# gersteinlab/LESSeq

Hardware: AMD Instinct MI355X
Metric: MRF reads/sec through count+solve (higher is better)
Workload: dtype int32 coordinates / u64 counters (count), f64 (EM); 1 GPU; BASELINE configs[2]: 100M synthetic 100bp reads over 50k mixed events (SE/RI/A5SS/A3SS/MXE/AFE/ALE/T3), 24 chromosomes; events=50000

## Files before the change

include/lesseq_hip.h:

```cpp
#ifndef LESSEQ_HIP_H
#define LESSEQ_HIP_H

#include <stddef.h>
#include <stdint.h>

#ifdef __cplusplus
extern "C" {
#endif

#define LSQ_ABI_VERSION 2

typedef enum {
	LSQ_OK = 0,
	LSQ_E_ARG = -1,
	LSQ_E_IO = -2,
	LSQ_E_FORMAT = -3,
	LSQ_E_PARSE = -4,
	LSQ_E_RANGE = -5,
	LSQ_E_UNSUPPORTED = -6,
	LSQ_E_DEVICE = -7,
	LSQ_E_STATE = -8,
	LSQ_E_INTERNAL = -9,
	LSQ_E_TIMEOUT = -10
} lsq_status;
// ... 38 lines not shown
const char *lsq_events_chrom(const lsq_events *e, int64_t ev);
const char *lsq_events_strand(const lsq_events *e, int64_t ev);
int lsq_events_num_isoforms(const lsq_events *e, int64_t ev);
int lsq_events_num_segments(const lsq_events *e, int64_t ev);
const char *lsq_events_isoform_name(const lsq_events *e, int64_t ev, int iso);
int lsq_events_segment(const lsq_events *e, int64_t ev, int n, int64_t *start, int64_t *end);
uint64_t lsq_events_isoform_mask(const lsq_events *e, int64_t ev, int iso);
uint64_t lsq_events_isoform_length(const lsq_events *e, int64_t ev, int iso);
uint64_t lsq_events_ars(const lsq_events *e, int method, int64_t ev, int iso);
int lsq_events_span(const lsq_events *e, int64_t ev, int64_t *gene_start, int64_t *gene_end);
int64_t lsq_events_num_buckets(const lsq_events *e);
int64_t lsq_events_lds_table_bytes(const lsq_events *e);
int64_t lsq_events_host_genes(const lsq_events *e);
int lsq_events_set_shard(lsq_events *e, uint64_t first_event, uint64_t n_events);

int lsq_mrf_parse(const char *read_format, const char *path, lsq_events *e,
                  int n_threads, lsq_reads **out);
int lsq_reads_parse(const char *read_format, const char *path, lsq_events *e, int n_threads, lsq_reads **out);
#define LSQ_SAM_DEFAULT_SKIP_FLAGS 0x904u
#define LSQ_SAM_DEFAULT_MIN_MAPQ 0u
int lsq_sam_parse(const char *path, lsq_events *e, unsigned skip_flags, unsigned min_mapq, int n_threads, lsq_reads **out);
int lsq_sam_to_mrf(const void *sam_bytes, uint64_t len, unsigned skip_flags, unsigned min_mapq, char **mrf_text, uint64_t *mrf_len);
int lsq_bam_parse(const char *path, lsq_events *e, unsigned skip_flags, unsigned min_mapq, int n_threads, lsq_reads **out);
int lsq_bam_to_mrf(const void *bam_bytes, uint64_t len, unsigned skip_flags, unsigned min_mapq, char **mrf_text, uint64_t *mrf_len);
int lsq_bam_parse_checked(const char *path, lsq_events *e, unsigned skip_flags, unsigned min_mapq, int n_threads, lsq_reads **out);
int lsq_bam_to_mrf_checked(const void *bam_bytes, uint64_t len, unsigned skip_flags, unsigned min_mapq, char **mrf_text, uint64_t *mrf_len);
typedef struct { uint64_t file_bytes, blocks, inflated_bytes, header_lines, references, records, reads, read_blocks, blocks_repaired; } lsq_bam_report;
int lsq_bam_check_host(const char *path, int n_threads, lsq_bam_report *r);
int lsq_reads_wrap(uint64_t n_reads, const uint64_t *blk_off, const uint32_t *line_no,
                   const int32_t *blk_start, const int32_t *blk_end,
                   const uint16_t *blk_chrom_id, const uint8_t *blk_strand_id, lsq_reads **out);
void lsq_reads_free(lsq_reads *r);
uint64_t lsq_reads_count(const lsq_reads *r);
uint64_t lsq_reads_num_blocks(const lsq_reads *r);
int lsq_events_chrom_id(lsq_events *e, const char *chrom);
int lsq_events_strand_id(lsq_events *e, const char *strand);
const char *lsq_events_strand_name(const lsq_events *e, int strand_id);
int lsq_reads_arrays(const lsq_reads *r, const uint64_t **blk_off, const uint32_t **line_no,
                     const int32_t **blk_start, const int32_t **blk_end,
                     const uint16_t **blk_chrom_id, const uint8_t **blk_strand_id);


typedef struct lsq_ctx lsq_ctx;

int lsq_ctx_create(int device_id, lsq_ctx **out);
#define LSQ_CTX_LANES_IN_BACKGROUND 1u
int lsq_ctx_create_with(int device_id, unsigned flags, lsq_ctx **out);
void lsq_ctx_destroy(lsq_ctx *c);
void *lsq_ctx_stream(lsq_ctx *c);
int lsq_ctx_synchronize(lsq_ctx *c);
int lsq_ctx_synchronize_for(lsq_ctx *c, double seconds);

int lsq_events_upload(lsq_ctx *c, lsq_events *e);

int lsq_reads_upload(lsq_ctx *c, int method, const lsq_reads *r);
int lsq_reads_upload_mrf(lsq_ctx *c, int method, const char *read_format, const char *path);
typedef struct lsq_text lsq_text;
int lsq_text_stage(lsq_ctx *c, const char *path, lsq_text **out);
void lsq_text_free(lsq_text *t);
int lsq_reads_upload_text(lsq_ctx *c, int method, const char *read_format, lsq_text *t);
int lsq_text_stage_range(lsq_ctx *c, const char *path, uint64_t byte_begin, uint64_t byte_end, lsq_text **out);
int lsq_text_lines(lsq_ctx *c, lsq_text *t, uint64_t *n_newlines);
int lsq_reads_upload_text_at(lsq_ctx *c, int method, const char *read_format, lsq_text *t, int has_header, uint64_t first_line);
int lsq_mrf_parse_device(lsq_ctx *c, const char *read_format, const char *path, lsq_reads **out);
int lsq_last_mrf_timing(lsq_ctx *c, float *h2d_ms, float *parse_ms);
int lsq_ingest_stage_count(void);
const char *lsq_ingest_stage_name(int stage);
int lsq_last_ingest_stages(const lsq_ctx *c, float *ms, uint64_t *bytes, int capacity);
const char *lsq_last_ingest_stage_name(const lsq_ctx *c, int stage);
int lsq_last_ingest_stage_count(const lsq_ctx *c);
int lsq_last_sam_paths(const lsq_ctx *c, uint32_t *lines_listed, uint32_t *all_slow);
int lsq_last_bam_paths(const lsq_ctx *c, uint64_t *n_blocks, uint64_t *blocks_repaired);
int lsq_bam_check(lsq_ctx *c, const char *path, lsq_bam_report *r);
uint64_t lsq_reads_retained(const lsq_ctx *c, int method);
int lsq_last_library_report(const lsq_ctx *c, int method, uint64_t out[5]);
uint64_t lsq_reads_retained_blocks(const lsq_ctx *c, int method);
uint64_t lsq_reads_pooled(const lsq_ctx *c, int method);
uint64_t lsq_reads_pooled_blocks(const lsq_ctx *c, int method);
int lsq_reads_pool_format(const lsq_ctx *c, int method, int *compact, uint64_t *pool_bytes, uint64_t *pool_reads);

int lsq_count(lsq_ctx *c);
int lsq_count_status(lsq_ctx *c, uint32_t *exceptions, uint32_t *recounted);
int lsq_count_launch_info(lsq_ctx *c, uint32_t *reads_per_look, uint32_t *workgroups_per_cu);
int lsq_host_evaluated(const lsq_ctx *c, uint64_t *n_genes, uint64_t *n_reads);
int lsq_ctx_set_option(lsq_ctx *c, const char *name, double value);

int lsq_solve(lsq_ctx *c);

int64_t lsq_results_num_classes(const lsq_ctx *c);
int lsq_results_class_offsets(const lsq_ctx *c, uint64_t *class_off );
int lsq_results_counts(lsq_ctx *c, uint64_t *class_count, uint64_t *class_bases);
int lsq_results_set_counts(lsq_ctx *c, const uint64_t *class_count, const uint64_t *class_bases);
uint64_t lsq_counts_device_words(const lsq_ctx *c);
int lsq_counts_export_device(lsq_ctx *c, void *d_words);
int lsq_counts_import_device(lsq_ctx *c, const void *d_words);
int lsq_results_solve(lsq_ctx *c, double *theta, double *logll, uint32_t *em_iters, uint8_t *em_flags);
int lsq_solve_finalize(lsq_ctx *c, uint32_t *n_replayed);
int lsq_set_em_guard_band(lsq_ctx *c, double band);

int lsq_fim(lsq_ctx *c);
int64_t lsq_results_fim_size(const lsq_ctx *c);
int lsq_results_fim_offsets(const lsq_ctx *c, uint64_t *fim_off );
int lsq_results_fim(lsq_ctx *c, double *fim, double *var_by_diag, double *var_by_inverse);

int lsq_results_copy_device(lsq_ctx *c, void *d_class_count, void *d_theta, void *d_logll);
void *lsq_ctx_result_stream(lsq_ctx *c);

int lsq_shard_bounds(const lsq_events *e, int world, const double *weights ,
                     uint64_t *first , uint64_t *count );
uint64_t lsq_record_words(const lsq_events *e, uint64_t first, uint64_t count);
int lsq_results_pack_device(lsq_ctx *c, void *d_block);
int lsq_device_alloc(lsq_ctx *c, uint64_t bytes, void **out);
void lsq_device_free(lsq_ctx *c, void *p);
int lsq_device_read(lsq_ctx *c, void *host_dst, const void *device_src, uint64_t bytes);
int lsq_device_write(lsq_ctx *c, void *device_dst, const void *host_src, uint64_t bytes);
int lsq_gathered_unpack(const lsq_events *e, int world, const uint64_t *first, const uint64_t *count,
                        const uint64_t *blocks, uint64_t stride_words,
                        uint64_t *class_count, uint64_t *class_bases, double *theta, double *logll);
int lsq_results_device_order(const lsq_ctx *c, int32_t *dev2out );

int lsq_set_timing(lsq_ctx *c, int on);
int lsq_last_timing(lsq_ctx *c, float *count_ms, float *solve_ms);
int lsq_last_fast_kernel_ms(lsq_ctx *c, float *ms);


int lsq_format_count(const lsq_events *e, int n_methods, const uint64_t *class_count, char **out_text);
int lsq_format_solve(const lsq_events *e, int n_methods, const uint64_t *class_count,
                     const uint64_t *class_bases, const double *theta, const double *logll,
                     const double *total_read_bases, char **out_text);
void lsq_free(void *p);

int lsq_cli_run(const char *tool, int argc, const char *const *argv, char **out_text);
int lsq_cli_main(const char *tool, int argc, const char *const *argv);


int lsq_as_fisher(lsq_ctx *c, uint64_t n_tables, const double *cells , double *p);
int lsq_as_lrt(lsq_ctx *c, uint64_t n_rows, int n1, int n2, const double *count, const double *total ,
               double *stat, double *p);
int lsq_as_wilcox(lsq_ctx *c, uint64_t n_rows, int n1, int n2, const double *value , double *diff, double *p);
int lsq_as_adjust(lsq_ctx *c, uint64_t n, const double *p, double *p_bonferroni, double *p_bh);

typedef struct lsq_as_input lsq_as_input;
int lsq_as_read_matrix(const char *test, int n_paths, const char *const *paths, int n1, int n2, lsq_as_input **out);
int lsq_as_read_tables(const char *test, int n_paths, const char *const *paths, int n1, int n2, lsq_as_input **out);
void lsq_as_input_free(lsq_as_input *in);
uint64_t lsq_as_input_rows(const lsq_as_input *in);
int lsq_as_input_columns(const lsq_as_input *in);
const char *lsq_as_input_id(const lsq_as_input *in, uint64_t row);
const double *lsq_as_input_values(const lsq_as_input *in);
const double *lsq_as_input_totals(const lsq_as_input *in);
uint64_t lsq_as_input_left_out(const lsq_as_input *in);
int lsq_as_format_number(double v, char *buf, size_t cap);


typedef struct lsq_jn_index lsq_jn_index;
typedef struct lsq_jn_table lsq_jn_table;
int lsq_jn_index_build(const lsq_annotation *a, lsq_jn_index **out);
void lsq_jn_index_free(lsq_jn_index *ix);
int64_t lsq_jn_index_num_chroms(const lsq_jn_index *ix);
const char *lsq_jn_index_chrom_name(const lsq_jn_index *ix, int64_t chrom);
int64_t lsq_jn_index_num_introns(const lsq_jn_index *ix);
lsq_events *lsq_jn_index_dictionaries(lsq_jn_index *ix);
int lsq_jn_host(lsq_jn_index *ix, const char *read_format, const char *path, unsigned skip_flags, unsigned min_mapq,
                uint32_t min_overhang, int n_threads, lsq_jn_table **out);
int lsq_jn_host_reads(lsq_jn_index *ix, const lsq_reads *r, uint32_t min_overhang, int n_threads, lsq_jn_table **out);
int lsq_jn_device(lsq_ctx *c, lsq_jn_index *ix, const char *read_format, const char *path, uint32_t min_overhang, lsq_jn_table **out);
// ... 69 lines not shown
```

include/lesseq_hip_dev.h:

```cpp
#ifndef LESSEQ_HIP_DEV_H
#define LESSEQ_HIP_DEV_H

#include <stdint.h>
#include "lesseq_hip.h"

#ifdef __cplusplus
extern "C" {
#endif

int lsq_debug_counters(lsq_ctx *c, unsigned long long *out16);
int lsq_debug_wg_trace(lsq_ctx *c, unsigned long long *out, unsigned long long cap, unsigned long long *n, unsigned long long *n_workers);

int lsq_debug_slot_offsets(lsq_ctx *c, int method, unsigned long long *out, unsigned long long n);
int lsq_debug_plan_shares(const unsigned long long *slot_off, const unsigned char *packed, const unsigned long long *n1, const unsigned long long *n2,
                          const unsigned *look1, const unsigned *look2, unsigned long long n_buckets, unsigned long long grid,
                          const double *costs4, int weighted, int snap, unsigned long long *cuts);
int lsq_debug_offsets(lsq_ctx *c, int method, int which, unsigned long long *out, unsigned long long cap, unsigned long long *n);

int lsq_debug_set_em_order(lsq_ctx *c, const uint32_t *order, unsigned n_small_places, unsigned n_places);

int lsq_debug_stream_read_rate(lsq_ctx *c, unsigned long long bytes, double *gb_per_s);

int lsq_debug_throw(int kind);

int lsq_debug_last_parse_paths(const lsq_ctx *c, unsigned *tiles_handed, unsigned *lines_listed, unsigned *all_slow);

int lsq_debug_bgzf_inflate(lsq_ctx *c, const void *bytes, uint64_t len, void *out, uint64_t cap, uint64_t *n);

int lsq_debug_bgzf_crc32(lsq_ctx *c, const void *bytes, uint64_t len, uint32_t *crc, uint64_t cap, uint64_t *n);

int lsq_debug_hip_versions(int *compiled, int *runtime);

int64_t lsq_debug_events_covered(const lsq_events *e, const char *chrom, int minus, int64_t *starts, int64_t *ends, int64_t capacity);

#ifdef __cplusplus
}
#endif
#endif
```

lesseq_amd/_lib.py:

```python
import ctypes as C
import os

_HERE = os.path.dirname(os.path.abspath(__file__))
LIB_PATH = os.environ.get("LSQ_LIB") or os.path.join(_HERE, "_build", "liblesseq_hip.so")


class LsqError(RuntimeError):
    def __init__(self, status, msg):
        super().__init__("lsq status %d: %s" % (status, msg))
        self.status = status


if not os.path.exists(LIB_PATH):
    raise ImportError("%s is missing: build it with `make -C lesseq_amd/csrc` (or __graft_entry__.build()); "
                      "there is no fallback implementation" % LIB_PATH)

if os.environ.get("LSQ_NO_TORCH") != "1":
    try:
        import torch
    except Exception:
        pass

lib = C.CDLL(LIB_PATH)

# ... 32 lines not shown
_sig("lsq_events_compile_library", C.c_int, vp, C.c_int, P(cs), P(u64), C.c_int, P(vp))
_sig("lsq_events_library", C.c_int, vp)
_sig("lsq_library_from_name", C.c_int, cs)
_sig("lsq_debug_events_covered", C.c_int64, vp, cs, C.c_int, P(C.c_int64), P(C.c_int64), C.c_int64)
_sig("lsq_events_free", None, vp)
_sig("lsq_events_count", i64, vp)
_sig("lsq_events_total_isoforms", i64, vp)
_sig("lsq_events_gene_name", cs, vp, i64)
_sig("lsq_events_chrom", cs, vp, i64)
_sig("lsq_events_strand", cs, vp, i64)
_sig("lsq_events_num_isoforms", C.c_int, vp, i64)
_sig("lsq_events_num_segments", C.c_int, vp, i64)
_sig("lsq_events_isoform_name", cs, vp, i64, C.c_int)
_sig("lsq_events_segment", C.c_int, vp, i64, C.c_int, P(i64), P(i64))
_sig("lsq_events_isoform_mask", u64, vp, i64, C.c_int)
_sig("lsq_events_isoform_length", u64, vp, i64, C.c_int)
_sig("lsq_events_ars", u64, vp, C.c_int, i64, C.c_int)
_sig("lsq_events_span", C.c_int, vp, i64, P(i64), P(i64))
_sig("lsq_events_num_buckets", i64, vp)
_sig("lsq_events_lds_table_bytes", i64, vp)
_sig("lsq_events_host_genes", i64, vp)
_sig("lsq_events_set_shard", C.c_int, vp, u64, u64)
_sig("lsq_mrf_parse", C.c_int, cs, cs, vp, C.c_int, P(vp))
_sig("lsq_reads_parse", C.c_int, cs, cs, vp, C.c_int, P(vp))
_sig("lsq_sam_parse", C.c_int, cs, vp, C.c_uint, C.c_uint, C.c_int, P(vp))
_sig("lsq_sam_to_mrf", C.c_int, cs, u64, C.c_uint, C.c_uint, P(vp), P(u64))
_sig("lsq_bam_parse", C.c_int, cs, vp, C.c_uint, C.c_uint, C.c_int, P(vp))
_sig("lsq_bam_to_mrf", C.c_int, cs, u64, C.c_uint, C.c_uint, P(vp), P(u64))
_sig("lsq_bam_parse_checked", C.c_int, cs, vp, C.c_uint, C.c_uint, C.c_int, P(vp))
_sig("lsq_bam_to_mrf_checked", C.c_int, cs, u64, C.c_uint, C.c_uint, P(vp), P(u64))
_sig("lsq_bam_check_host", C.c_int, cs, C.c_int, P(BamReportStruct))
_sig("lsq_reads_wrap", C.c_int, u64, P(u64), P(u32), P(i32), P(i32), P(u16), P(u8), P(vp))
_sig("lsq_reads_free", None, vp)
_sig("lsq_reads_count", u64, vp)
_sig("lsq_reads_num_blocks", u64, vp)
_sig("lsq_events_chrom_id", C.c_int, vp, cs)
_sig("lsq_events_strand_id", C.c_int, vp, cs)
_sig("lsq_ctx_create", C.c_int, C.c_int, P(vp))
_sig("lsq_ctx_destroy", None, vp)
_sig("lsq_ctx_stream", vp, vp)
_sig("lsq_ctx_synchronize", C.c_int, vp)
_sig("lsq_ctx_synchronize_for", C.c_int, vp, C.c_double)
_sig("lsq_debug_throw", C.c_int, C.c_int)
_sig("lsq_debug_hip_versions", C.c_int, P(C.c_int), P(C.c_int))
_sig("lsq_events_upload", C.c_int, vp, vp)
_sig("lsq_reads_upload", C.c_int, vp, C.c_int, vp)
_sig("lsq_reads_arrays", C.c_int, vp, P(vp), P(vp), P(vp), P(vp), P(vp), P(vp))
_sig("lsq_events_strand_name", cs, vp, C.c_int)
_sig("lsq_reads_upload_mrf", C.c_int, vp, C.c_int, cs, cs)
_sig("lsq_text_stage", C.c_int, vp, cs, P(vp))
_sig("lsq_text_stage_range", C.c_int, vp, cs, u64, u64, P(vp))
_sig("lsq_text_lines", C.c_int, vp, vp, P(u64))
_sig("lsq_reads_upload_text_at", C.c_int, vp, C.c_int, cs, vp, C.c_int, u64)
_sig("lsq_results_set_counts", C.c_int, vp, P(u64), P(u64))
_sig("lsq_text_free", None, vp)
_sig("lsq_reads_upload_text", C.c_int, vp, C.c_int, cs, vp)
_sig("lsq_mrf_parse_device", C.c_int, vp, cs, cs, P(vp))
_sig("lsq_last_mrf_timing", C.c_int, vp, P(C.c_float), P(C.c_float))
_sig("lsq_set_log_level", None, C.c_int)
_sig("lsq_ingest_stage_count", C.c_int)
_sig("lsq_ingest_stage_name", cs, C.c_int)
_sig("lsq_last_ingest_stages", C.c_int, vp, P(C.c_float), P(u64), C.c_int)
_sig("lsq_last_ingest_stage_name", cs, vp, C.c_int)
_sig("lsq_last_sam_paths", C.c_int, vp, P(u32), P(u32))
_sig("lsq_last_ingest_stage_count", C.c_int, vp)
_sig("lsq_last_bam_paths", C.c_int, vp, P(u64), P(u64))
_sig("lsq_debug_bgzf_inflate", C.c_int, vp, cs, u64, vp, u64, P(u64))
_sig("lsq_debug_bgzf_crc32", C.c_int, vp, cs, u64, P(u32), u64, P(u64))
_sig("lsq_bam_check", C.c_int, vp, cs, P(BamReportStruct))
_sig("lsq_reads_retained", u64, vp, C.c_int)
_sig("lsq_last_library_report", C.c_int, vp, C.c_int, P(u64))
_sig("lsq_reads_retained_blocks", u64, vp, C.c_int)
_sig("lsq_reads_pooled", u64, vp, C.c_int)
_sig("lsq_reads_pooled_blocks", u64, vp, C.c_int)
_sig("lsq_reads_pool_format", C.c_int, vp, C.c_int, C.POINTER(C.c_int), C.POINTER(C.c_uint64), C.POINTER(C.c_uint64))
_sig("lsq_count", C.c_int, vp)
_sig("lsq_solve", C.c_int, vp)
_sig("lsq_results_num_classes", i64, vp)
_sig("lsq_results_class_offsets", C.c_int, vp, P(u64))
_sig("lsq_results_counts", C.c_int, vp, P(u64), P(u64))
_sig("lsq_results_solve", C.c_int, vp, P(C.c_double), P(C.c_double), P(u32), P(u8))
_sig("lsq_count_status", C.c_int, vp, P(u32), P(u32))
_sig("lsq_count_launch_info", C.c_int, vp, P(u32), P(u32))
_sig("lsq_host_evaluated", C.c_int, vp, P(u64), P(u64))
_sig("lsq_counts_device_words", u64, vp)
_sig("lsq_counts_export_device", C.c_int, vp, vp)
_sig("lsq_counts_import_device", C.c_int, vp, vp)
_sig("lsq_ctx_set_option", C.c_int, vp, cs, C.c_double)
_sig("lsq_solve_finalize", C.c_int, vp, P(u32))
_sig("lsq_set_em_guard_band", C.c_int, vp, C.c_double)
_sig("lsq_results_copy_device", C.c_int, vp, vp, vp, vp)
_sig("lsq_ctx_result_stream", vp, vp)
_sig("lsq_shard_bounds", C.c_int, vp, C.c_int, P(C.c_double), P(u64), P(u64))
_sig("lsq_record_words", u64, vp, u64, u64)
_sig("lsq_results_pack_device", C.c_int, vp, vp)
_sig("lsq_gathered_unpack", C.c_int, vp, C.c_int, P(u64), P(u64), P(u64), u64, P(u64), P(u64), P(C.c_double), P(C.c_double))
_sig("lsq_device_alloc", C.c_int, vp, u64, P(vp))
_sig("lsq_device_free", None, vp, vp)
_sig("lsq_device_read", C.c_int, vp, vp, vp, u64)
_sig("lsq_device_write", C.c_int, vp, vp, vp, u64)
_sig("lsq_results_device_order", C.c_int, vp, P(i32))
_sig("lsq_fim", C.c_int, vp)
_sig("lsq_results_fim_size", C.c_int64, vp)
_sig("lsq_results_fim_offsets", C.c_int, vp, P(C.c_uint64))
_sig("lsq_results_fim", C.c_int, vp, P(C.c_double), P(C.c_double), P(C.c_double))
_sig("lsq_set_timing", C.c_int, vp, C.c_int)
_sig("lsq_last_fast_kernel_ms", C.c_int, vp, P(C.c_float))
_sig("lsq_last_timing", C.c_int, vp, P(C.c_float), P(C.c_float))
_sig("lsq_format_count", C.c_int, vp, C.c_int, P(u64), P(vp))
_sig("lsq_format_solve", C.c_int, vp, C.c_int, P(u64), P(u64), P(C.c_double), P(C.c_double), P(C.c_double), P(vp))
_sig("lsq_cli_run", C.c_int, cs, C.c_int, P(cs), P(vp))
_sig("lsq_synth_write", C.c_int, P(SynthSpecStruct), cs, cs, C.c_int)
_sig("lsq_synth_write_sam", C.c_int, P(SynthSpecStruct), cs, cs)
_sig("lsq_as_fisher", C.c_int, vp, u64, P(C.c_double), P(C.c_double))
_sig("lsq_as_lrt", C.c_int, vp, u64, C.c_int, C.c_int, P(C.c_double), P(C.c_double), P(C.c_double), P(C.c_double))
_sig("lsq_as_wilcox", C.c_int, vp, u64, C.c_int, C.c_int, P(C.c_double), P(C.c_double), P(C.c_double))
_sig("lsq_as_adjust", C.c_int, vp, u64, P(C.c_double), P(C.c_double), P(C.c_double))
_sig("lsq_as_read_matrix", C.c_int, cs, C.c_int, P(cs), C.c_int, C.c_int, P(vp))
_sig("lsq_as_read_tables", C.c_int, cs, C.c_int, P(cs), C.c_int, C.c_int, P(vp))
_sig("lsq_as_input_free", None, vp)
_sig("lsq_as_input_rows", u64, vp)
_sig("lsq_as_input_columns", C.c_int, vp)
_sig("lsq_as_input_id", cs, vp, u64)
_sig("lsq_as_input_values", P(C.c_double), vp)
_sig("lsq_as_input_totals", P(C.c_double), vp)
_sig("lsq_as_input_left_out", u64, vp)
_sig("lsq_as_format_number", C.c_int, C.c_double, C.c_char_p, C.c_size_t)
_sig("lsq_synth_reads", C.c_int, P(SynthSpecStruct), vp, C.c_int, P(vp))
_sig("lsq_le_load_matrices", C.c_int, cs, cs, P(vp))
_sig("lsq_le_load_annotation", C.c_int, cs, cs, cs, cs, P(vp))
_sig("lsq_le_graphs_free", None, vp)
_sig("lsq_le_num_genes", i64, vp)
_sig("lsq_le_gene_name", cs, vp, i64)
_sig("lsq_le_gene_shape", C.c_int, vp, i64, P(C.c_int), P(C.c_int))
_sig("lsq_le_gene_positions", i64, vp, i64, P(P(i32)))
_sig("lsq_le_detect", C.c_int, vp, vp, P(vp))
_sig("lsq_le_result_free", None, vp)
_sig("lsq_le_type_name", cs, C.c_int)
_sig("lsq_le_num_events", i64, vp, C.c_int)
_sig("lsq_le_event", C.c_int, vp, C.c_int, i64, P(i64), P(i32))
_sig("lsq_le_format", C.c_int, vp, C.c_int, P(vp), P(vp))
_sig("lsq_le_result_times", C.c_int, vp, P(C.c_double))
_sig("lsq_le_write", C.c_int, vp, cs)
_sig("lsq_gtf_parse", C.c_int, vp, cs, P(vp))
_sig("lsq_gtf_parse_text", C.c_int, vp, cs, u64, P(vp))
_sig("lsq_gtf_free", None, vp)
_sig("lsq_gtf_num_transcripts", i64, vp)
_sig("lsq_gtf_num_genes", i64, vp)
_sig("lsq_gtf_num_exon_lines", i64, vp)
_sig("lsq_gtf_transcript_name", cs, vp, i64)
_sig("lsq_gtf_transcript_chrom", cs, vp, i64)
_sig("lsq_gtf_transcript_strand", cs, vp, i64)
_sig("lsq_gtf_transcript_exons", i64, vp, i64, P(P(i32)), P(P(i32)))
_sig("lsq_gtf_format", C.c_int, vp, P(vp), P(vp))
_sig("lsq_gtf_result_times", C.c_int, vp, P(C.c_double))
_sig("lsq_gtf_isoform_map", C.c_int, cs, u64, P(vp))
_sig("lsq_le_load_gtf", C.c_int, vp, cs, P(vp))
_sig("lsq_jn_index_build", C.c_int, vp, P(vp))
_sig("lsq_jn_index_free", None, vp)
_sig("lsq_jn_index_num_chroms", i64, vp)
_sig("lsq_jn_index_chrom_name", cs, vp, i64)
_sig("lsq_jn_index_num_introns", i64, vp)
_sig("lsq_jn_index_dictionaries", vp, vp)
_sig("lsq_jn_host", C.c_int, vp, cs, cs, C.c_uint, C.c_uint, u32, C.c_int, P(vp))
_sig("lsq_jn_host_reads", C.c_int, vp, vp, u32, C.c_int, P(vp))
_sig("lsq_jn_device", C.c_int, vp, vp, cs, cs, u32, P(vp))
# ... 36 lines not shown
```

lesseq_amd/api.py:

```python
import os
import ctypes as C

import numpy as np

from ._lib import lib, check, check_runtime_once, SynthSpecStruct, BamReportStruct, u64, u32, i32, u16, u8, i64, vp, cs, P

EVENT_TYPES = ("SE", "RI", "A5SS", "A3SS", "MXE", "AFE", "ALE", "T3")


def _b(s):
    return s.encode() if isinstance(s, str) else s


def _take_text(ptr):
    if not ptr:
        return ""
    s = C.string_at(ptr).decode()
    lib.lsq_free(ptr)
    return s


def _ptr(a, ct):
    return a.ctypes.data_as(P(ct))

# ... 327 lines not shown
            out = (u32 * cap)()
            st = lib.lsq_debug_bgzf_crc32(self.h, data, len(data), out, cap, C.byref(n))
            if st == -5 and n.value > cap:
                cap = n.value
                continue
            check(st)
            return [int(v) for v in out[:n.value]]

    def bam_check(self, path):
        r = BamReportStruct()
        check(lib.lsq_bam_check(self.h, _b(path), C.byref(r)))
        return _bam_report(r)

    def mrf_timing(self):
        a, b = C.c_float(), C.c_float()
        check(lib.lsq_last_mrf_timing(self.h, C.byref(a), C.byref(b)))
        return {"h2d_ms": a.value, "parse_ms": b.value}

    def parse_paths(self):
        a, b, c = C.c_uint(), C.c_uint(), C.c_uint()
        lib.lsq_debug_last_parse_paths.argtypes = [vp, P(C.c_uint), P(C.c_uint), P(C.c_uint)]
        lib.lsq_debug_last_parse_paths.restype = C.c_int
        check(lib.lsq_debug_last_parse_paths(self.h, C.byref(a), C.byref(b), C.byref(c)))
        return {"tiles_to_byte_walking_kernel": a.value, "lines_to_shared_splitter": b.value, "whole_file_byte_walking": bool(c.value)}

    def ingest_stages(self):
        n = lib.lsq_last_ingest_stage_count(self.h)
        ms, by = (C.c_float * n)(), (C.c_uint64 * n)()
        check(lib.lsq_last_ingest_stages(self.h, ms, by, n))
        return [{"stage": lib.lsq_last_ingest_stage_name(self.h, i).decode(), "ms": float(ms[i]), "bytes": int(by[i])} for i in range(n)]

    def retained(self, method):
        return lib.lsq_reads_retained(self.h, method)

    def library_report(self, method=0):
        out = (u64 * 5)()
        check(lib.lsq_last_library_report(self.h, method, out))
        return tuple(out)

    def pooled(self, method):
        return lib.lsq_reads_pooled(self.h, method)

    def pooled_blocks(self, method):
        return lib.lsq_reads_pooled_blocks(self.h, method)

    def pool_format(self, method):
        a, n = C.c_int(0), C.c_uint64(0)
        k = (C.c_uint64 * 3)()
        check(lib.lsq_reads_pool_format(self.h, method, C.byref(a), C.byref(n), k))
        return bool(a.value), n.value, tuple(int(x) for x in k)

    def retained_blocks(self, method):
        return lib.lsq_reads_retained_blocks(self.h, method)

    def count(self):
        check(lib.lsq_count(self.h))

    def solve(self):
        check(lib.lsq_solve(self.h))

    def set_option(self, name, value):
        check(lib.lsq_ctx_set_option(self.h, _b(name), float(value)))

    def count_status(self):
        M = max(self.events.n_methods, 1)
        e, r = (u32 * M)(), (u32 * M)()
        check(lib.lsq_count_status(self.h, e, r))
        return list(e)[:self.events.n_methods], list(r)[:self.events.n_methods]

    def counts_device_words(self):
        return int(lib.lsq_counts_device_words(self.h))

    def export_counts_device(self, d_ptr):
        check(lib.lsq_counts_export_device(self.h, vp(d_ptr)))

    def import_counts_device(self, d_ptr):
        check(lib.lsq_counts_import_device(self.h, vp(d_ptr)))

    def launch_info(self):
        a, b = u32(), u32()
        check(lib.lsq_count_launch_info(self.h, C.byref(a), C.byref(b)))
        return int(a.value), int(b.value)

    def set_em_guard_band(self, band):
        check(lib.lsq_set_em_guard_band(self.h, float(band)))

    def solve_finalize(self):
        n = u32()
        check(lib.lsq_solve_finalize(self.h, C.byref(n)))
        return n.value

    def synchronize(self):
        check(lib.lsq_ctx_synchronize(self.h))

    @property
    def stream(self):
        return lib.lsq_ctx_stream(self.h)

    def set_timing(self, on=True):
        check(lib.lsq_set_timing(self.h, 1 if on else 0))

    def timing(self):
        a, b = C.c_float(), C.c_float()
        check(lib.lsq_last_timing(self.h, C.byref(a), C.byref(b)))
        return a.value, b.value

    def copy_results_device(self, d_class_count=None, d_theta=None, d_logll=None):
        check(lib.lsq_results_copy_device(self.h, vp(d_class_count), vp(d_theta), vp(d_logll)))

    def pack_results_device(self, d_block):
        check(lib.lsq_results_pack_device(self.h, vp(d_block)))

    @property
    def result_stream(self):
        return lib.lsq_ctx_result_stream(self.h)

    def device_order(self):
        o = np.zeros(max(len(self.events), 1), np.int32)
        check(lib.lsq_results_device_order(self.h, _ptr(o, i32)))
        return o[:len(self.events)]

    def fast_kernel_ms(self):
        a = C.c_float()
        check(lib.lsq_last_fast_kernel_ms(self.h, C.byref(a)))
        return a.value

    def counts(self):
        n = lib.lsq_results_num_classes(self.h)
        M = self.events.n_methods
        cnt = np.zeros((max(M, 1), max(n, 1)), np.uint64)
        bases = np.zeros((max(M, 1), max(n, 1)), np.uint64)
        check(lib.lsq_results_counts(self.h, _ptr(cnt, u64), _ptr(bases, u64)))
        return cnt[:M, :n], bases[:M, :n]

    def set_counts(self, cnt, bases):
        cnt = np.ascontiguousarray(cnt, np.uint64)
        bases = np.ascontiguousarray(bases, np.uint64)
        check(lib.lsq_results_set_counts(self.h, _ptr(cnt, u64), _ptr(bases, u64)))

    def stage_text(self, path, byte_begin=0, byte_end=2 ** 64 - 1):
        h = vp()
        check(lib.lsq_text_stage_range(self.h, _b(path), byte_begin, byte_end, C.byref(h)))
        return h

    def text_lines(self, text):
        n = u64()
        check(lib.lsq_text_lines(self.h, text, C.byref(n)))
        return n.value

    def upload_reads_text(self, method, text, has_header=True, first_line=1, read_format="MRF_SINGLE", free=True):
        try:
            check(lib.lsq_reads_upload_text_at(self.h, method, _b(read_format), text, 1 if has_header else 0, first_line))
        finally:
            if free:
                lib.lsq_text_free(text)

    def solution(self):
        ne, ni = len(self.events), self.events.total_isoforms
        theta = np.zeros(max(ni, 1), np.float64)
        ll = np.zeros(max(ne, 1), np.float64)
        it = np.zeros(max(ne, 1), np.uint32)
        fl = np.zeros(max(ne, 1), np.uint8)
        check(lib.lsq_results_solve(self.h, _ptr(theta, C.c_double), _ptr(ll, C.c_double), _ptr(it, u32), _ptr(fl, u8)))
        return theta[:ni], ll[:ne], it[:ne], fl[:ne]

    def fim(self):
# ... 54 lines not shown
```

lesseq_amd/csrc/lsq_count.hip:

```cpp
#include "lsq_device.hpp"
#include <hip/hip_ext.h>

namespace {

#ifndef LSQ_COUNT_BLOCK
#define LSQ_COUNT_BLOCK 256
#endif
constexpr int COUNT_BLOCK = LSQ_COUNT_BLOCK;
constexpr unsigned long long BASES_MASK = (1ull << 40) - 1;

#ifdef LSQ_DEV
#define ABL(args, bits) ((((args).ablate) & (bits)) != 0u)
#else
#define ABL(args, bits) false
#endif


struct CountArgs {
	const BucketDesc *buckets;
	const unsigned char *images;
	const TieRec *ties;
	const unsigned char *strand_rank;
	const char *read_names; const unsigned long long *read_name_off;
	const char *gene_names; const unsigned *gene_name_off;
	unsigned n_buckets;
	unsigned ablate;
	unsigned tables_lds_bytes;
	const void *p1; const unsigned char *p1_strand; const unsigned *p1_line;
	const void *p2; const unsigned char *p2_strand; const unsigned *p2_line;
	unsigned compact;
	const unsigned *pn_blk_off; const unsigned *pn_nblk; const int2 *pn_se; const unsigned char *pn_strand; const unsigned *pn_line; const unsigned *pn_bucket;
	const unsigned long long *p1_off, *p2_off, *pn_off, *slot_off;
	const lsq::VisitRec *visits;
	const unsigned *wg_first;
	const unsigned long long *wg_cut;
	const lsq::WgPlan *wg_plan;
	unsigned long long *wg_trace;
	unsigned long long total_slots;
	unsigned long long n_pn;
	unsigned n_workers;
	unsigned long long *cnt, *bases;
	struct ExcEntry *exc;
	unsigned *exc_count;
	unsigned exc_cap;
	unsigned long long *dbg;
	unsigned long long *bar;
};

__device__ inline int2 unpack_one_block(const unsigned a, const int base) {
	const int s = base + (int)(a & lsq::COMPACT_OFF_MASK);
	return make_int2(s, s + (int)(a >> lsq::COMPACT_OFF_BITS));
}
__device__ inline int4 unpack_two_block(const unsigned a, const unsigned b, const int base) {
	const int s1 = base + (int)(a & lsq::COMPACT_OFF_MASK), e1 = s1 + (int)(a >> lsq::COMPACT_OFF_BITS);
	const int s2 = e1 + (int)(b & lsq::COMPACT_OFF_MASK);
	return make_int4(s1, e1, s2, s2 + (int)(b >> lsq::COMPACT_OFF_BITS));
}
__device__ inline int2 pool1_read(const CountArgs &A, const unsigned long long g, const int lo) {
	if (!A.compact) return reinterpret_cast<const int2 *>(A.p1)[g];
	return unpack_one_block(reinterpret_cast<const unsigned *>(A.p1)[g], lo - lsq::COMPACT_BIAS);
}
__device__ inline int4 pool2_read(const CountArgs &A, const unsigned long long g, const int lo) {
	if (!A.compact) return reinterpret_cast<const int4 *>(A.p2)[g];
	const uint2 v = reinterpret_cast<const uint2 *>(A.p2)[g];
	return unpack_two_block(v.x, v.y, lo - lsq::COMPACT_BIAS);
}

struct LdsView {
	const unsigned short *bins;
	const EventRec *ev;
	const int2 *segs;
	const unsigned *iso;
	unsigned long long *hist;
};

__device__ __noinline__ bool tie_orders_read_first(const CountArgs &A, unsigned ev_index, unsigned read_strand, unsigned line) {
	const TieRec *t = A.ties + ev_index;
	const unsigned rs = A.strand_rank[read_strand], gs = A.strand_rank[t->strand_id];
	if (rs != gs) return rs < gs;
	if (A.read_name_off) {
		const unsigned long long r0 = A.read_name_off[line], r1 = A.read_name_off[line + 1];
		const unsigned g0 = A.gene_name_off[ev_index], g1 = A.gene_name_off[ev_index + 1];
		const unsigned long long rn = r1 - r0;
		const unsigned gn = g1 - g0;
		for (unsigned long long i = 0; i < rn && i < gn; ++i) {
			const unsigned char a = (unsigned char)A.read_names[r0 + i], b = (unsigned char)A.gene_names[g0 + i];
			if (a != b) return a < b;
		}
		return rn < gn;
	}
	const unsigned mode = t->tie_mode;
	if (mode != 2) return mode == 1;
	unsigned pow10 = 1, nd = 1;
	while (nd < 10 && line / pow10 >= 10) { pow10 *= 10; ++nd; }
	const unsigned tl = t->tail_len;
	unsigned v = line;
	for (unsigned i = 0; i < nd && i < tl; ++i) {
		const unsigned char a = (unsigned char)('0' + v / pow10), b = (unsigned char)t->tail[i];
		if (a != b) return a < b;
		v %= pow10; pow10 /= 10;
	}
	return nd < tl;
}

struct Walk {
	int pos = 0, it = 0;
	bool found = false;
	unsigned mask = 0;
	int matched = 0;
	__device__ inline bool block(const int2 *segs, int nseg, int a, int b) {
		while (it < nseg) {
// ... 468 lines not shown
					const bool inside1 = v1 && !start1 && rd.y <= (int)cw1.z && rd.z != rd.y;
					const bool ends1 = inside1 && rd.y == (int)cw1.z;
					const unsigned ri = 3u * (v1 ? cx1.w : 0u);
					const uint4 w0r = C.recs[ri], w1r = C.recs[ri + 1u], w2r = C.recs[ri + 2u];
					const unsigned k2 = rd.z == (int)w1r.z ? 1u : (rd.z == (int)w2r.x ? 2u : (rd.z == (int)w2r.z ? 3u : 0u));
					const int end2 = k2 == 1u ? (int)w1r.w : (k2 == 2u ? (int)w2r.y : (int)w2r.w);
					const bool cont = ends1 && k2 > k1;
					const bool J = cont && rd.w <= end2;
					const bool S = inside1 && !cont;
					const bool drop = (v1 && start1 && rd.w <= (int)cw1.w) || (here && i1 == CELL_INFO_EMPTY);
					const unsigned len1 = (unsigned)(rd.y - rd.x), total = len1 + (unsigned)(rd.w - rd.z);
					const unsigned long long tbl = ((unsigned long long)w0r.w << 32) | w0r.z;
					const unsigned cls = (unsigned)(tbl >> (4u * ((1u << (k1 & 3u)) | (1u << k2)))) & 0xFu;
					const unsigned sa = cx1.x & 0xFFFFu;
					L.junction = cont;
					L.jslot = cls != 0u ? (w0r.y & 0xFFFFu) + cls - 1u : CELL_NONE;
					L.add = in && ((J && cls != 0u) || (S && sa != CELL_NONE && 50u * len1 > 49u * total));
					L.slot = J ? (w0r.y & 0xFFFFu) + cls - 1u : sa;
					L.matched = J ? total : len1;
					L.park = in && !(J || S || drop);
					L.hint = v1 ? (cx1.w | PARK_ONE_EVENT) : evf;
					L.c = make_int4((int)cw1.x, (int)cw1.y, 0, end2);
					if (ABL(A, 256u) && L.park) atomicAdd(&A.dbg[8 + (v1 ? 1 : 0)], 1ull);
					return L;
				};
				const uint4 u = cur[0];
				const int4 rd = make_int4((int)u.x, (int)u.y, (int)u.z, (int)u.w);
				const unsigned w0i = wt + lane * (unsigned)SW;
				const unsigned rel = w0i - first_rel;
				const bool in = w0i < ww1 && rel < n_rel;
				const Look L1 = look2(rd, in);
				unsigned n_add = L1.add ? 1u : 0u, s_add = L1.add ? L1.matched : 0u, n_add2 = 0, s_add2 = 0;
				park[0] = L1.park && !ABL(A, 17u | 1048576u);
				pe0[0] = uint4(u);
				pe1[0] = make_uint4(L1.hint, rel, 0u, 0u);
#pragma unroll
				for (int j = 1; j < N_READS; ++j) {
					const uint4 &v = cur[j];
					const int4 r2 = make_int4((int)v.x, (int)v.y, (int)v.z, (int)v.w);
					const unsigned wj = wt + lane * (unsigned)SW + (unsigned)j;
					const unsigned rel2 = wj - first_rel;
					const bool in2 = wj < ww1 && rel2 < n_rel;
					const bool same = in2 && L1.junction && r2.y == rd.y && r2.z == rd.z && L1.c.x <= r2.x && r2.x < L1.c.y && r2.w <= L1.c.w;
					n_add2 += (same && L1.jslot != CELL_NONE) ? 1u : 0u;
					s_add2 += (same && L1.jslot != CELL_NONE) ? (unsigned)((r2.y - r2.x) + (r2.w - r2.z)) : 0u;
					park[j] = in2 && !same && r2.y != r2.x && !ABL(A, 17u | 1048576u | 2097152u);
					pe0[j] = uint4(v);
					pe1[j] = make_uint4(PARK_EVENT_UNKNOWN, rel2, 0u, 0u);
				}
				if (!ABL(A, 1u)) {
					if (n_add && n_add2 && L1.slot == L1.jslot) { n_add += n_add2; s_add += s_add2; n_add2 = 0; }
					if (n_add) atomicAdd(&C.hist[L1.slot], ((unsigned long long)n_add << 40) | s_add);
					if (n_add2) atomicAdd(&C.hist[L1.jslot], ((unsigned long long)n_add2 << 40) | s_add2);
				} else asm volatile("" ::"v"(n_add), "v"(s_add), "v"(n_add2), "v"(s_add2));
			}
		}
		if (RPW == 1) {
			static_assert(RPW != 1 || N_READS == 2, "two parked entries a step");
#pragma unroll
			for (int q = 0; q < 2; ++q) {
				const bool pq = park[q ? N_READS - 1 : 0];
				const uint4 q0 = pe0[q ? N_READS - 1 : 0], q1 = pe1[q ? N_READS - 1 : 0];
				if (ABL(A, 256u) && pq) atomicAdd(&A.dbg[NB - 1], 1ull);
				R.push(pq, lane, q0, q1);
				if (R.live() >= 64u) {
					if (!ABL(A, 32u)) walk_parked<NB>(C, R, false);
					else R.head = R.tail;
				}
			}
		}
	};
	if (ww0 < ww1) fetch(ww0);
	for (unsigned wt = ww0; wt < ww1; wt += WAVES * TILE) {
		uint4 cur[SW];
#pragma unroll
		for (int k = 0; k < SW; ++k) cur[k] = nxt[k];
		if (wt + WAVES * TILE < ww1) fetch(wt + WAVES * TILE);
		do_step(cur, wt);
	}
	if (R.live() && !ABL(A, 32u)) walk_parked<NB>(C, R, true);
}


template <int NR>
__device__ inline void stream_pool1_compact(FastCtx &C, const uint4 *bins, const uint4 *cells, const uint4 *cellx, const unsigned n_cells, const BucketDesc &d,
                                            const CountArgs &A, uint4 *queue, const void *pool, const unsigned long long g0, const unsigned long long g1) {
	static_assert(NR == 4 || NR == 8, "one or two 16-byte words of four compact records");
	static_assert((unsigned)NR <= P1_GROUP_PAD, "a lane's records of a step lie in one cell group");
	constexpr int CW = NR / 4;
	constexpr unsigned TILE = 64u * NR;
	C.pool = 0u;
	C.slot0 = g0;
	global_words src = (global_words)pool;
	const unsigned lane = threadIdx.x & 63u, wave = (unsigned)__builtin_amdgcn_readfirstlane((int)(threadIdx.x >> 6));
	const unsigned long long R0 = g0 & ~(unsigned long long)(NR - 1);
	const unsigned n = (unsigned)(g1 - R0), first_rel = (unsigned)(g0 - R0), n_rel = (unsigned)(g1 - g0);
	const unsigned last_word = (n - 1u) >> 2;
	const int base = d.lo - lsq::COMPACT_BIAS;
	uint4 nxt[CW];
	auto fetch = [&](const unsigned t) {
#pragma unroll
		for (int cq = 0; cq < CW; ++cq) {
			const unsigned w = min((t >> 2) + lane * (unsigned)CW + (unsigned)cq, last_word);
			const u32x4 v = src[(R0 >> 2) + w];
			nxt[cq] = make_uint4(v.x, v.y, v.z, v.w);
		}
	};
	Ring<1> R;
	R.q = queue;
	const unsigned t_begin = min(wave * TILE, n);
	if (t_begin < n) fetch(t_begin);
	for (unsigned t = t_begin; t < n; t += WAVES * TILE) {
		unsigned rec[NR];
#pragma unroll
		for (int cq = 0; cq < CW; ++cq) { rec[4 * cq] = nxt[cq].x; rec[4 * cq + 1] = nxt[cq].y; rec[4 * cq + 2] = nxt[cq].z; rec[4 * cq + 3] = nxt[cq].w; }
		if (t + WAVES * TILE < n) fetch(t + WAVES * TILE);
		if (ABL(A, 512u)) {
#pragma unroll
			for (int j = 0; j < NR; ++j) asm volatile("" ::"v"(rec[j]));
			continue;
		}
		const int p0 = (int)(rec[0] & lsq::COMPACT_OFF_MASK) + base;
		const int rel0 = p0 - d.lo;
		const unsigned bin = rel0 <= 0 ? 0u : ((unsigned)rel0 >> d.shift);
		const uint4 br = bins[min(bin, d.n_bins - 1u)];
		unsigned ci = (br.x & 0xFFFFu) + (unsigned)(p0 >= (int)br.y) + (unsigned)(p0 >= (int)br.z) + (unsigned)(p0 >= (int)br.w);
		if (__any(p0 >= (int)br.w) && !ABL(A, 65536u)) {
			while (ci + 1u < n_cells && p0 >= (int)cells[ci + 1u].x) ++ci;
		}
		const unsigned cc = min(ci, n_cells - 1u);
		const uint4 cw = cells[cc];
		const uint4 cx = cellx[cc];
		const bool has = ci < n_cells && (int)cw.x <= p0 && p0 < (int)cw.y && !ABL(A, 8u);
		const bool both = has && (cx.z & CELLX_BOTH) != 0;
		const int e1 = has ? (int)cw.z - base : -1, e2 = has ? (int)cw.w - base : -1;
		const bool interior = t + TILE <= n && t >= first_rel;
		unsigned accN = 0, accA = 0, accL = 0;
		auto decide = [&](auto whole_step, auto one_threshold) {
#pragma unroll
			for (int j = 0; j < NR; ++j) {
				const unsigned len = rec[j] >> lsq::COMPACT_OFF_BITS;
				const int e = (int)(rec[j] & lsq::COMPACT_OFF_MASK) + (int)len;
				unsigned p = len | (min(len, 1u) << 24);
				if (!decltype(whole_step)::value) {
					const unsigned idx = t + lane * (unsigned)NR + (unsigned)j;
					p = (idx < n && idx - first_rel < n_rel) ? p : 0u;
				}
				accN += p;
				accA += e <= e1 ? p : 0u;
				if (!decltype(one_threshold)::value) accL += e <= e2 ? p : 0u;
			}
			if (decltype(one_threshold)::value) accL = accA;
		};
		if (__all(e1 == e2) && !ABL(A, 8388608u)) { if (interior) decide(std::true_type{}, std::true_type{}); else decide(std::false_type{}, std::true_type{}); }
		else { if (interior) decide(std::true_type{}, std::false_type{}); else decide(std::false_type{}, std::false_type{}); }
		const unsigned s1 = cx.x & 0xFFFFu, s2 = cx.x >> 16;
		if (!ABL(A, (1u | 16384u))) {
			const unsigned acc2 = both ? accL : accL - accA;
			if (accA && s1 != CELL_NONE) atomicAdd(&C.hist[s1], ((unsigned long long)(accA >> 24) << 40) | (accA & 0xFFFFFFu));
			if (acc2 && s2 != CELL_NONE) atomicAdd(&C.hist[s2], ((unsigned long long)(acc2 >> 24) << 40) | (acc2 & 0xFFFFFFu));
		} else asm volatile("" ::"v"(accA), "v"(accL));
		const bool lane_open = (accN >> 24) != ((both ? accA : accL) >> 24);
		if (ABL(A, 256u)) {
			const bool any_open = __any(lane_open);
			if (lane == 0) { atomicAdd(&A.dbg[12], 1ull); atomicAdd(&A.dbg[11], any_open ? 1ull : 0ull); }
		}
		if (__any(lane_open) && !ABL(A, 17u | 524288u)) {
#pragma unroll
			for (int h = 0; h < NR; h += 2) {
				uint4 en[2];
				unsigned open = 0;
#pragma unroll
				for (int j = h; j < h + 2; ++j) {
					const unsigned len = rec[j] >> lsq::COMPACT_OFF_BITS;
					const int so = (int)(rec[j] & lsq::COMPACT_OFF_MASK), e = so + (int)len;
					const unsigned idx = t + lane * (unsigned)NR + (unsigned)j, rel = idx - first_rel;
					const bool in = idx < n && rel < n_rel;
					const bool gone_near = both && (cx.z & CELLX_NEAR_NO_ABUT) != 0u && e > e1 && 50 * (e - e1) >= (int)len;
					const bool gone_far = both && (cx.z & CELLX_FAR_NO_ABUT) != 0u && e > e2 && 50 * (e - e2) >= (int)len;
					const bool done_near = e <= e1 || gone_near, done_far = e <= e2 || gone_far;
					const bool op = in && len != 0u && !(both ? (done_near && done_far) : e <= e2);
					open |= op ? 1u << (j - h) : 0u;
					const unsigned hint = !has ? PARK_EVENT_UNKNOWN : (!both ? (cx.w | PARK_ONE_EVENT) :
					                      (done_far ? (cx.w | PARK_ONE_EVENT) : (done_near ? ((cx.z & 0xFFFFu) | PARK_ONE_EVENT) : PARK_EVENT_UNKNOWN)));
					en[j - h] = make_uint4((unsigned)(so + base), (unsigned)(so + base) + len, hint, rel);
					if (ABL(A, 256u) && op) { atomicAdd(&A.dbg[5 + (has ? (both ? 2 : 1) : 0)], 1ull); atomicAdd(&A.dbg[0], 1ull); }
				}
				R.push2(open, lane, en[0], en[1]);
				if (R.live() >= 64u) {
					if (!ABL(A, 32u)) walk_parked<1, false>(C, R, false, base);
					else R.head = R.tail;
				}
			}
		}
	}
	if (R.live() && !ABL(A, 32u)) walk_parked<1, false>(C, R, true, base);
}

template <int NR>
__device__ inline void stream_pool2_compact(FastCtx &C, const uint4 *bins, const uint4 *cells, const uint4 *cellx, const unsigned n_cells, const BucketDesc &d,
                                            const CountArgs &A, uint4 *queue, const void *pool, const unsigned long long g0, const unsigned long long g1) {
	static_assert((NR == 2 || NR == 4 || NR == 8) && (unsigned)NR <= P2_GROUP_PAD, "whole 16-byte words of two compact records, inside one junction group");
	constexpr int CW = NR / 2;
	constexpr unsigned TILE = 64u * NR;
	C.pool = 1u;
	C.slot0 = g0;
	global_words src = (global_words)pool;
	const unsigned lane = threadIdx.x & 63u, wave = (unsigned)__builtin_amdgcn_readfirstlane((int)(threadIdx.x >> 6));
	const unsigned long long R0 = g0 & ~(unsigned long long)(NR - 1);
	const unsigned n = (unsigned)(g1 - R0), first_rel = (unsigned)(g0 - R0), n_rel = (unsigned)(g1 - g0);
	const unsigned last_word = (n - 1u) >> 1;
	const int base = d.lo - lsq::COMPACT_BIAS;
	uint4 nxt[CW];
	auto fetch = [&](const unsigned t) {
#pragma unroll
		for (int cq = 0; cq < CW; ++cq) {
			const unsigned w = min((t >> 1) + lane * (unsigned)CW + (unsigned)cq, last_word);
			const u32x4 v = src[(R0 >> 1) + w];
			nxt[cq] = make_uint4(v.x, v.y, v.z, v.w);
		}
	};
	Ring<1> R;
	R.q = queue;
	const unsigned t_begin = min(wave * TILE, n);
	if (t_begin < n) fetch(t_begin);
	for (unsigned t = t_begin; t < n; t += WAVES * TILE) {
		unsigned ra[NR], rb[NR];
#pragma unroll
		for (int cq = 0; cq < CW; ++cq) { ra[2 * cq] = nxt[cq].x; rb[2 * cq] = nxt[cq].y; ra[2 * cq + 1] = nxt[cq].z; rb[2 * cq + 1] = nxt[cq].w; }
		if (t + WAVES * TILE < n) fetch(t + WAVES * TILE);
		if (ABL(A, 512u)) {
#pragma unroll
			for (int j = 0; j < NR; ++j) asm volatile("" ::"v"(ra[j]), "v"(rb[j]));
			continue;
		}
		const bool interior = t + TILE <= n && t >= first_rel;
		const unsigned idx0 = t + lane * (unsigned)NR, rel0 = idx0 - first_rel;
		const bool in0 = interior || (idx0 < n && rel0 < n_rel);
		const int4 rd = unpack_two_block(ra[0], rb[0], base);
		const int rel_p = rd.x - d.lo;
		const unsigned bin = rel_p <= 0 ? 0u : ((unsigned)rel_p >> d.shift);
		const uint4 br = bins[min(bin, d.n_bins - 1u)];
		unsigned c1 = (br.x & 0xFFFFu) + (unsigned)(rd.x >= (int)br.y) + (unsigned)(rd.x >= (int)br.z) + (unsigned)(rd.x >= (int)br.w);
		const unsigned evf = br.x >> 16;
		if (__any(rd.x >= (int)br.w) && !ABL(A, 65536u)) {
			while (c1 + 1u < n_cells && rd.x >= (int)cells[c1 + 1u].x) ++c1;
		}
		const unsigned c1c = min(c1, n_cells - 1u);
		const uint4 cw1 = cells[c1c];
		const uint4 cx1 = cellx[c1c];
		const unsigned i1 = cx1.y;
		const unsigned k1 = (i1 >> 2) & 0x3Fu;
		const bool here = c1 < n_cells && (int)cw1.x <= rd.x && rd.x < (int)cw1.y && !ABL(A, 8u);
		const bool v1 = here && i1 < CELL_INFO_EMPTY;
		const bool start1 = k1 == CELL_K_START;
		const bool inside1 = v1 && !start1 && rd.y <= (int)cw1.z && rd.z != rd.y;
		const bool ends1 = inside1 && rd.y == (int)cw1.z;
		const bool ends1b = v1 && !start1 && (int)cw1.w > (int)cw1.z && rd.y == (int)cw1.w && rd.z != rd.y;
		const unsigned ri = 3u * (v1 ? cx1.w : 0u);
		const uint4 w0r = C.recs[ri], w1r = C.recs[ri + 1u], w2r = C.recs[ri + 2u];
		const unsigned k2 = rd.z == (int)w1r.z ? 1u : (rd.z == (int)w2r.x ? 2u : (rd.z == (int)w2r.z ? 3u : 0u));
		const int end2 = k2 == 1u ? (int)w1r.w : (k2 == 2u ? (int)w2r.y : (int)w2r.w);
		const unsigned abut = (w0r.y >> FAST_ABUT_SHIFT) & 7u;
		const bool abut2 = k2 != 0u && k2 < 3u && ((abut >> k2) & 1u) != 0u;
		const int end2b = !abut2 ? end2 : (k2 == 1u ? (int)w2r.y : (int)w2r.w);
		const unsigned k1e = ends1b ? k1 + 1u : k1;
		const bool junction = (ends1 || ends1b) && k2 > k1e;
		const bool J = junction && rd.w <= end2, Jb = junction && rd.w > end2 && rd.w <= end2b;
		const unsigned len1 = ra[0] >> lsq::COMPACT_OFF_BITS, total = len1 + (rb[0] >> lsq::COMPACT_OFF_BITS);
		const unsigned long long tbl = ((unsigned long long)w0r.w << 32) | w0r.z;
		const unsigned mask1 = (1u << (k1 & 3u)) | (ends1b ? 2u << (k1 & 3u) : 0u), maskA = mask1 | (1u << k2), maskB = maskA | (2u << k2);
		const unsigned clsA = (unsigned)(tbl >> (4u * (maskA & 15u))) & 0xFu, clsB = abut2 ? (unsigned)(tbl >> (4u * (maskB & 15u))) & 0xFu : 0u;
		const unsigned sa = cx1.x & 0xFFFFu;
		const unsigned slotA = clsA != 0u ? (w0r.y & 0xFFFFu) + clsA - 1u : CELL_NONE, slotB = clsB != 0u ? (w0r.y & 0xFFFFu) + clsB - 1u : CELL_NONE;
		const bool any_plain = __any(!junction);
		bool two = false, empty = false, near_free = false, far_free = false, S = false, drop = false, addS = false;
		int e1c = 0, e2c = 0;
// ... 67 lines not shown
		}
	}
	if (R.live() && !ABL(A, 32u)) walk_parked<2, true>(C, R, true, base);
}

__device__ inline void global_add_merged(unsigned long long *cnt, unsigned long long *bases, bool want, const unsigned slot, const unsigned matched) {
	const unsigned lane = threadIdx.x & 63u;
#pragma unroll 1
	for (int round = 0; round < 4; ++round) {
		const unsigned long long m = __ballot(want);
		if (!m) return;
		const unsigned lead = (unsigned)__ffsll((long long)m) - 1u;
		const unsigned s0 = (unsigned)__builtin_amdgcn_readlane((int)slot, lead);
		const bool same = want && slot == s0;
		const unsigned n = (unsigned)__popcll(__ballot(same));
		const unsigned sum = wave_sum_u32(same ? matched : 0u);
		if (lane == lead) { atomicAdd(&cnt[s0], (unsigned long long)n); atomicAdd(&bases[s0], (unsigned long long)sum); }
		want = want && !same;
	}
	if (want) { atomicAdd(&cnt[slot], 1ull); atomicAdd(&bases[slot], (unsigned long long)matched); }
}

__device__ inline void pool_n_worker(const CountArgs &A, const unsigned long long n_pn, const unsigned n_workers) {
	const unsigned long long gsz = (unsigned long long)n_workers * COUNT_BLOCK;
	for (unsigned long long g0 = (unsigned long long)blockIdx.x * COUNT_BLOCK; g0 < n_pn; g0 += gsz) {
		const unsigned long long g = g0 + threadIdx.x;
		bool active = g < n_pn;
		const unsigned b = active ? A.pn_bucket[g] : 0u;
		const BucketDesc *d = A.buckets + b;
		active = active && d->kind == 1;
		const unsigned *bins = reinterpret_cast<const unsigned *>(A.images + d->img_off);
		const uint4 *recs = reinterpret_cast<const uint4 *>(A.images + d->img_off + d->ev_off);
		const int2 *blk = A.pn_se + (active ? A.pn_blk_off[g] : 0u);
		const int nblk = active ? (int)A.pn_nblk[g] : 1;
		int p = 0, q = 0, total = 0;
		unsigned i = 0;
		if (active) {
			p = blk[0].x; q = blk[nblk - 1].y;
			for (int k = 0; k < nblk; ++k) total += blk[k].y - blk[k].x;
			const int rel = p - d->lo;
			const unsigned bin = rel <= 0 ? 0u : min((unsigned)rel >> d->shift, d->n_bins - 1u);
			i = bins[4u * bin] >> 16;
		}
		while (__any(active)) {
			bool want = false;
			unsigned slot = 0, matched = 0;
			if (active) {
				if (i >= d->n_events) active = false;
				else {
					const uint4 w0 = recs[3u * i];
					const int2 *segs = reinterpret_cast<const int2 *>(recs + 3u * i + 1u);
					const int gs = segs[0].x, ge = (int)w0.x;
					if (gs > p) active = false;
					else {
						bool cand = p <= ge;
						if (cand && p == gs) {
							if (q == ge) {
								const unsigned at = atomicAdd(A.exc_count, 1u);
								if (at < A.exc_cap) { ExcEntry e; e.slot = g; e.bucket = b; e.ev_pool_scan = i | (2u << 29); A.exc[at] = e; }
							}
							cand = q > ge;
						}
						if (cand) {
							const int nseg = (int)((w0.y >> FAST_NSEG_SHIFT) & 7u);
							Walk w;
							for (int k = 0; k < nblk; ++k) { const int2 bk = blk[k]; if (!w.block(segs, nseg, bk.x, bk.y)) break; }
							const unsigned long long tbl = ((unsigned long long)w0.w << 32) | w0.z;
							const unsigned cls = w.mask < 16u ? (unsigned)(tbl >> (4u * w.mask)) & 0xFu : 0u;
							if (cls != 0 && 50ll * w.matched > 49ll * total) { want = true; slot = d->cls_base + (w0.y & 0xFFFFu) + cls - 1; matched = (unsigned)w.matched; }
						}
						if (p <= ge && !(w0.y & FAST_FLAG_OVERLAPS_NEXT)) active = false;
						++i;
					}
				}
			}
			global_add_merged(A.cnt, A.bases, want, slot, matched);
		}
	}
}

#ifndef LSQ_FAST_WAVES
#define LSQ_FAST_WAVES 6
#endif
template <bool COMPACT, int P1W>
__global__ void __launch_bounds__(COUNT_BLOCK, P1W == 4 ? 5 : LSQ_FAST_WAVES) lsq_count_fast_kernel(CountArgs A) {
	extern __shared__ __align__(16) unsigned char lds[];
	const unsigned tid = threadIdx.x;
	struct Trace {
		unsigned long long *p;
		__device__ Trace(unsigned long long *q) : p(q) { if (p && threadIdx.x == 0) p[4u * blockIdx.x] = wall_clock64(); }
		__device__ ~Trace() { if (p && threadIdx.x == 0) p[4u * blockIdx.x + 1u] = wall_clock64(); }
	} trace(ABL(A, 4194304u) ? A.wg_trace : nullptr);
	if (blockIdx.x < A.n_workers) { pool_n_worker(A, A.n_pn, A.n_workers); return; }
	const unsigned wg = blockIdx.x - A.n_workers, n_wg = gridDim.x - A.n_workers;
	uint4 *wave_queue = reinterpret_cast<uint4 *>(lds + A.tables_lds_bytes) + (tid >> 6) * WAVE_QUEUE_WORDS;
	(void)n_wg;
	typedef const lsq::VisitRec __attribute__((address_space(4))) *const_visit;
	typedef const lsq::WgPlan __attribute__((address_space(4))) *const_plan;
	const_plan plan = (const_plan)(A.wg_plan + wg);
	const unsigned long long s_begin = plan->s_begin, s_end = plan->s_end;
	if (s_begin >= s_end) return;
	if (ABL(A, 4096u)) return;
	const_visit vr = &plan->first;
	unsigned b = vr->b;
	bool first_visit = true;
	while (b < A.n_buckets) {
		const unsigned long long bs = vr->bs;
		if (bs >= s_end) break;
		BucketDesc d;
		d.img_off = vr->d.img_off; d.img_bytes = vr->d.img_bytes; d.n_events = vr->d.n_events; d.n_bins = vr->d.n_bins; d.lo = vr->d.lo; d.shift = vr->d.shift;
		d.ev_off = vr->d.ev_off; d.seg_off = vr->d.seg_off; d.iso_off = vr->d.iso_off; d.hist_off = vr->d.hist_off; d.n_cls = vr->d.n_cls; d.cls_base = vr->d.cls_base;
		d.ev_base = vr->d.ev_base; d.chrom_id = vr->d.chrom_id; d.kind = vr->d.kind; d.hi = vr->d.hi;
		const unsigned long long be = vr->be, p1o = vr->p1o, n1 = vr->p1n, p2o = vr->p2o, n2 = vr->p2n;
		const unsigned next = vr->next;
		unsigned char *buf = lds;
		if (!first_visit) __syncthreads();
		first_visit = false;
		{
			global_words src = (global_words)(A.images + d.img_off);
			uint4 *dst = reinterpret_cast<uint4 *>(buf);
			for (unsigned i = tid; i < d.img_bytes / 16; i += COUNT_BLOCK) { const u32x4 t = src[i]; dst[i] = make_uint4(t.x, t.y, t.z, t.w); }
			unsigned long long *h = reinterpret_cast<unsigned long long *>(buf + d.hist_off);
			for (unsigned i = tid; i < HIST_REPLICAS * (d.n_cls | 1u); i += COUNT_BLOCK) h[i] = 0;
		}
		__syncthreads();
		if (ABL(A, 8192u)) return;
		const uint4 *bins = reinterpret_cast<const uint4 *>(buf);
		const uint4 *cells = reinterpret_cast<const uint4 *>(buf + d.seg_off);
		const unsigned n_cells = d.iso_off & 0xFFFFu;
		const uint4 *cellx = reinterpret_cast<const uint4 *>(buf + d.seg_off + 16u * (d.iso_off >> 16));
		FastCtx C;
		C.bins = bins; C.lo = d.lo; C.shift = d.shift; C.n_bins = d.n_bins;
		C.recs = reinterpret_cast<const uint4 *>(buf + d.ev_off);
		C.hist = reinterpret_cast<unsigned long long *>(buf + d.hist_off) + (tid & (HIST_REPLICAS - 1u)) * (d.n_cls | 1u);
		C.n_events = d.n_events; C.bucket = b;
		C.slot0 = 0; C.pool = 0;
		C.exc = A.exc; C.exc_count = A.exc_count; C.exc_cap = A.exc_cap; C.ablate = A.ablate; C.dbg = A.dbg;
		C.trace = (ABL(A, 4194304u) && A.wg_trace) ? A.wg_trace + 4u * blockIdx.x : nullptr;
		const unsigned long long l0 = (s_begin > bs ? s_begin : bs) - bs;
		const unsigned long long l1 = (s_end < be ? s_end : be) - bs;
		if (l0 < n1 && !ABL(A, 1024u)) {
			if constexpr (COMPACT) stream_pool1_compact<2 * P1W>(C, bins, cells, cellx, n_cells, d, A, wave_queue, A.p1, p1o + l0, p1o + (l1 < n1 ? l1 : n1));
			else stream_pool_wide<2>(C, bins, cells, cellx, n_cells, d, A, wave_queue, reinterpret_cast<const uint4 *>(A.p1), p1o + l0, p1o + (l1 < n1 ? l1 : n1));
		}
		if (l1 > n1 && l0 < n1 + n2 && !ABL(A, 2048u)) {
			const unsigned long long q0 = p2o + ((l0 > n1 ? l0 : n1) - n1), q1 = p2o + ((l1 < n1 + n2 ? l1 : n1 + n2) - n1);
			if constexpr (COMPACT) stream_pool2_compact<(P1W == 4 ? LSQ_P2_COMPACT_WORDS_W5 : LSQ_P2_COMPACT_WORDS)>(C, bins, cells, cellx, n_cells, d, A, wave_queue, A.p2, q0, q1);
			else stream_pool_wide<1>(C, bins, cells, cellx, n_cells, d, A, wave_queue, reinterpret_cast<const uint4 *>(A.p2), q0, q1);
		}
		__syncthreads();
		for (unsigned i = tid; i < d.n_cls; i += COUNT_BLOCK) {
			const unsigned long long *h0 = reinterpret_cast<const unsigned long long *>(buf + d.hist_off) + i;
			unsigned long long v = 0;
#pragma unroll
			for (unsigned r = 0; r < HIST_REPLICAS; ++r) v += h0[r * (d.n_cls | 1u)];
			if (v && !ABL(A, 4u)) {
				atomicAdd(&A.cnt[d.cls_base + i], v >> 40);
				atomicAdd(&A.bases[d.cls_base + i], v & BASES_MASK);
			}
		}
		if (be >= s_end) break;
		b = next;
		vr = (const_visit)(A.visits + b);
	}
}

struct GlobalBucket {
	const BucketDesc *d;
	const unsigned *bins;
	const uint4 *recs;
};

__device__ inline GlobalBucket global_bucket(const CountArgs &A, unsigned b) {
	GlobalBucket G;
	G.d = A.buckets + b;
	G.bins = reinterpret_cast<const unsigned *>(A.images + G.d->img_off);
	G.recs = reinterpret_cast<const uint4 *>(A.images + G.d->img_off + G.d->ev_off);
	return G;
}

__device__ void eval_read_global(const CountArgs &A, const GlobalBucket &G, const int2 *blk, int nblk, unsigned i, bool scan,
                                 unsigned strand_id, unsigned line) {
	const BucketDesc &d = *G.d;
	const int p = blk[0].x, q = blk[nblk - 1].y;
	int total = 0;
	for (int k = 0; k < nblk; ++k) total += blk[k].y - blk[k].x;
	for (; i < d.n_events; ++i) {
		const uint4 w0 = G.recs[3u * i], w1 = G.recs[3u * i + 1], w2 = G.recs[3u * i + 2];
		const int gs = (int)w1.x, ge = (int)w0.x;
		if (gs > p) break;
		bool cand = p <= ge;
		if (cand && p == gs) {
			if (q < ge) cand = false;
			else if (q == ge && tie_orders_read_first(A, d.ev_base + i, strand_id, line)) cand = false;
		}
		if (cand) {
			int2 segs[4] = {make_int2((int)w1.x, (int)w1.y), make_int2((int)w1.z, (int)w1.w), make_int2((int)w2.x, (int)w2.y), make_int2((int)w2.z, (int)w2.w)};
			const int nseg = (int)((w0.y >> FAST_NSEG_SHIFT) & 7u);
			Walk w;
			for (int k = 0; k < nblk; ++k) { const int2 bk = blk[k]; if (!w.block(segs, nseg, bk.x, bk.y)) break; }
			const unsigned long long tbl = ((unsigned long long)w0.w << 32) | w0.z;
			const unsigned cls = w.mask < 16u ? (unsigned)(tbl >> (4u * w.mask)) & 0xFu : 0u;
			if (cls != 0 && 50ll * w.matched > 49ll * total) {
				const unsigned slot = d.cls_base + (w0.y & 0xFFFFu) + cls - 1;
				atomicAdd(&A.cnt[slot], 1ull);
				atomicAdd(&A.bases[slot], (unsigned long long)(unsigned)w.matched);
			}
		}
		if (!scan) break;
		if (p <= ge && !(w0.y & FAST_FLAG_OVERLAPS_NEXT)) break;
	}
}

__device__ inline unsigned first_event_for(const GlobalBucket &G, int p) {
	const BucketDesc &d = *G.d;
	const int rel = p - d.lo;
	unsigned bin = rel <= 0 ? 0u : ((unsigned)rel >> d.shift);
	bin = min(bin, d.n_bins - 1u);
	return G.bins[4u * bin] >> 16;
}

__device__ void recount_all_reads(const CountArgs &A, unsigned long long n_pn);

__global__ void __launch_bounds__(256) lsq_count_cleanup_kernel(const CountArgs *Ap, int force_recount, unsigned long long n_pn,
                                                                const ExcEntry *exc, const unsigned *exc_count, unsigned exc_cap) {
// ... 89 lines not shown
	}
	for (size_t b = 0; b <= B; ++b) cum_b[b] = cum[std::min<size_t>(bseg[b], S)];
	const double total_cost = cum[S];
	const double wsum = (double)grid * (1.0 + taper) / 2.0;
	auto part_before = [&](unsigned long long g) {
		const double k = (double)g, slope = grid > 1 ? (taper - 1.0) / (double)(grid - 1) : 0.0;
		return (k + slope * k * (k - 1.0) / 2.0) / wsum;
	};
	size_t bb = 0, si = 0;
	for (unsigned long long g = 1; g < grid && total_cost > 0; ++g) {
		const double tc = total_cost * part_before(g), share = total_cost * (part_before(g + 1) - part_before(g));
		while (bb + 1 < B && cum_b[bb + 1] <= tc) ++bb;
		while (si + 1 < S && cum[si + 1] <= tc) ++si;
		const double xb = tc - cum_b[bb], yb = cum_b[bb + 1] - tc;
		unsigned long long t;
		if (pc.snap && xb <= yb && xb < 0.3 * share) t = so[bb];
		else if (pc.snap && yb < xb && yb < 0.3 * share) t = so[bb + 1];
		else {
			const double r = tc - cum[si] - jump[si];
			const unsigned long long len = x[si + 1] - x[si];
			t = x[si] + (r <= 0.0 ? 0ull : std::min<unsigned long long>((unsigned long long)(r / dens[si]), len));
		}
		cut[(size_t)g] = std::max(t, cut[(size_t)g - 1]);
	}
	if (!(total_cost > 0)) for (unsigned long long g = 1; g < grid; ++g) cut[(size_t)g] = total_slots * g / grid;
	cut[(size_t)grid] = total_slots;
	for (unsigned long long g = 0; g < grid; ++g)
		if (cut[(size_t)g + 1] - cut[(size_t)g] > (1ull << 21)) {
			for (unsigned long long q = 1; q < grid; ++q) cut[(size_t)q] = total_slots * q / grid;
			break;
		}
}

void plan_share_cuts(const unsigned long long *so, const unsigned char *visited_kind, const unsigned long long *pn1, const unsigned long long *pn2,
                     const unsigned *look1, const unsigned *look2, const size_t B, const unsigned long long grid, const SharePlanCosts &pc, unsigned long long *cut) {
	if (!(pc.weighted && pn1 && pn2 && look1 && look2)) { plan_share_cuts_seg(so, visited_kind, B, nullptr, nullptr, nullptr, nullptr, 0, grid, pc, cut); return; }
	std::vector<unsigned long long> x; std::vector<unsigned char> kind; std::vector<unsigned> looks, bseg(B + 1, 0);
	for (size_t b = 0; b < B; ++b) {
		bseg[b] = (unsigned)kind.size();
		const unsigned long long ns = so[b + 1] - so[b];
		if (!ns) continue;
		const bool visited = visited_kind[b] != 0;
		const unsigned long long n1 = visited ? std::min(pn1[b], ns) : 0, n2 = visited ? std::min(pn2[b], ns - n1) : 0;
		if (n1) { x.push_back(so[b]); kind.push_back(0); looks.push_back(look1[b]); }
		if (n2) { x.push_back(so[b] + n1); kind.push_back(1); looks.push_back(look2[b]); }
		if (ns - n1 - n2) { x.push_back(so[b] + n1 + n2); kind.push_back(2); looks.push_back(0); }
	}
	bseg[B] = (unsigned)kind.size();
	x.push_back(B ? so[B] : 0);
	plan_share_cuts_seg(so, visited_kind, B, x.data(), kind.data(), looks.data(), bseg.data(), kind.size(), grid, pc, cut);
}

int run_count(lsq_ctx *c) {
	const lsq_events &E = *c->E;
	const size_t n_cls = E.n_cls_total;
	const int M = E.n_methods;
	hipStream_t st_em = nullptr;
	const int set = c->flip ^ 1, other = c->flip;
	hipStream_t st = c->opt_two_count_streams ? c->stream_count2[set] : c->stream;
	if (c->mark_recorded2[set]) HIP_TRY(hipStreamWaitEvent(st, c->ev_mark2[set], 0));
	HIP_TRY(hipMemsetAsync(c->counters.p + (size_t)other * c->counters_per_set, 0, c->counters_per_set * sizeof(unsigned long long), c->stream_em2[other]));
	HIP_TRY(hipEventRecord(c->ev_mark2[other], c->stream_em2[other]));
	c->mark_recorded2[other] = true;
	select_counter_set(c, set);
	st_em = c->stream_em;
	c->fast_launched = 0;
	struct Cleanup { CountArgs A; unsigned long long n_pn; int m; };
	std::vector<Cleanup> cleanups;
	bool counted_signalled = false;
	if (c->time_events) HIP_TRY(hipEventRecord(c->ev0, st));
	const unsigned generic_tables_bytes = (std::max<unsigned>(E.max_lds_bytes, 16) + 15u) & ~15u;
	const unsigned tables_bytes = generic_tables_bytes;
	double max_skew = 0.0;
	for (int m = 0; m < M; ++m) max_skew = std::max(max_skew, c->reads[m].skew);
	const unsigned cap = c->opt_wg_per_cu >= 0 ? (unsigned)c->opt_wg_per_cu : (c->em_small_places >= c->opt_em_flat_min && max_skew < 4.0 ? 5u : 0u);
	const unsigned lds_bytes = std::max(tables_bytes + WAVES * WAVE_QUEUE_WORDS * 16, cap ? 160u * 1024u / (cap + 1u) + 16u : 0u);
	if (lds_bytes > 160 * 1024) return fail(LSQ_E_UNSUPPORTED, "bucket tables + read tile exceed the CU's LDS");
	bool all_compact = true;
	for (int m = 0; m < M; ++m) if (c->reads[m].total_slots && !c->reads[m].compact) all_compact = false;
	const int p1w = !all_compact ? 2 : (c->opt_reads_per_look ? (c->opt_reads_per_look == 8 ? 4 : 2) : (cap != 0 && cap <= 5 ? 4 : 2));
	const void *const fn_wide = (const void *)lsq_count_fast_kernel<false, 2>;
	const void *const fn_compact = p1w == 4 ? (const void *)lsq_count_fast_kernel<true, 4> : (const void *)lsq_count_fast_kernel<true, 2>;
	c->last_reads_per_look = 2u * (unsigned)p1w;
	if (lds_bytes > 64 * 1024) {
		HIP_TRY(hipFuncSetAttribute(fn_wide, hipFuncAttributeMaxDynamicSharedMemorySize, (int)lds_bytes));
		HIP_TRY(hipFuncSetAttribute(fn_compact, hipFuncAttributeMaxDynamicSharedMemorySize, (int)lds_bytes));
		HIP_TRY(hipFuncSetAttribute((const void *)lsq_count_generic_kernel, hipFuncAttributeMaxDynamicSharedMemorySize, (int)lds_bytes));
	}
	unsigned per_cu = std::max(1u, std::min(2048u / COUNT_BLOCK, (160u * 1024u) / lds_bytes));
	{
		if (c->occ_lds_bytes != lds_bytes || c->occ_p1w != p1w) {
			int nb = 0;
			int nb2 = 0;
			HIP_TRY(hipOccupancyMaxActiveBlocksPerMultiprocessor(&nb, fn_wide, (int)COUNT_BLOCK, (size_t)lds_bytes));
			HIP_TRY(hipOccupancyMaxActiveBlocksPerMultiprocessor(&nb2, fn_compact, (int)COUNT_BLOCK, (size_t)lds_bytes));
			c->occ_lds_bytes = lds_bytes; c->occ_p1w = p1w; c->occ_blocks = all_compact ? nb2 : std::min(nb, nb2);
		}
		if (c->occ_blocks >= 1) per_cu = std::min(per_cu, (unsigned)c->occ_blocks);
	}
	c->last_wg_per_cu = per_cu;
	for (int m = 0; m < M; ++m) {
		MethodReads &mr = c->reads[m];
		if (mr.total_slots == 0 || E.buckets.empty()) continue;
		const double mult = c->opt_grid_mult > 0 ? c->opt_grid_mult : (mr.skew >= 32.0 ? 4.0 : (mr.skew >= 4.0 || p1w == 4 ? 3.0 : 2.0));
		unsigned long long grid = (unsigned long long)((double)c->n_cu * per_cu * mult);
		grid = std::max(grid, mr.total_slots / (1ull << 21) + 1);
		grid = std::min<unsigned long long>(grid, std::max<unsigned long long>(mr.total_slots / 64, 1));
#ifdef LSQ_DEV
		if (const char *e = getenv("LSQ_GRID_WGS")) { const long v = atol(e); if (v >= 1) grid = (unsigned long long)v; }
#endif
		if (mr.wg_grid != grid) {
			const std::vector<unsigned long long> &so = mr.slot_off_host;
			const size_t B = E.buckets.size();
			std::vector<unsigned long long> cut((size_t)grid + 1, 0);
			std::vector<unsigned> first((size_t)grid, 0);
			const bool weighted = c->opt_share_weighted && mr.plan_n1.size() == B && mr.plan_park1.size() == B;
			SharePlanCosts pc;
			pc.weighted = weighted; pc.snap = c->opt_snap_shares;
			pc.two_block = c->opt_share_cost_p2; pc.walk_look = c->opt_share_cost_park; pc.visit = c->opt_share_cost_visit;
			pc.taper = c->opt_share_taper > 0 ? c->opt_share_taper : (mr.skew >= 4.0 ? 0.25 : 0.5);
			pc.hot = c->opt_share_cost_hot;
			std::vector<unsigned char> visited(B, 0);
			for (size_t q = 0; q < B; ++q) visited[q] = E.buckets[q].kind == 1u ? 1 : 0;
			if (weighted && mr.plan_seg_x.size() >= 2 && mr.plan_seg_first.size() == B + 1)
				plan_share_cuts_seg(so.data(), visited.data(), B, mr.plan_seg_x.data(), mr.plan_seg_kind.data(), mr.plan_seg_looks.data(), mr.plan_seg_first.data(),
				                    mr.plan_seg_kind.size(), grid, pc, cut.data());
			else
				plan_share_cuts(so.data(), visited.data(), weighted ? mr.plan_n1.data() : nullptr, weighted ? mr.plan_n2.data() : nullptr,
				                weighted ? mr.plan_park1.data() : nullptr, weighted ? mr.plan_park2.data() : nullptr, B, grid, pc, cut.data());
			size_t bb = 0;
			for (unsigned long long g = 0; g < grid; ++g) {
				while (bb + 1 < B && so[bb + 1] <= cut[(size_t)g]) ++bb;
				const unsigned f = mr.next_packed_host[bb];
				first[(size_t)g] = (f < B && so[f] < cut[(size_t)g + 1]) ? f : (unsigned)B;
			}
			int rc = mr.wg_first.upload(first.data(), first.size(), st);
			if (!rc) rc = mr.wg_cut.upload(cut.data(), cut.size(), st);
			if (rc) return rc;
			{
				std::vector<WgPlan> plan((size_t)grid);
				for (unsigned long long g = 0; g < grid; ++g) {
					WgPlan &w = plan[(size_t)g];
					w.s_begin = cut[(size_t)g]; w.s_end = cut[(size_t)g + 1];
					w.first = mr.visits_host[std::min<size_t>(first[(size_t)g], B)];
				}
				if ((rc = mr.wg_plan.upload(plan.data(), plan.size(), st))) return rc;
				HIP_TRY(hipStreamSynchronize(st));
			}
			HIP_TRY(hipStreamSynchronize(st));
			mr.wg_grid = grid;
		}
		CountArgs A{};
		A.buckets = c->buckets.p; A.images = c->images.p; A.ties = c->ties.p; A.strand_rank = c->strand_rank.p;
		A.wg_first = mr.wg_first.p; A.wg_cut = mr.wg_cut.p; A.wg_plan = mr.wg_plan.p; A.visits = mr.visits.p;
		A.read_names = mr.named ? mr.names.p : nullptr; A.read_name_off = mr.named ? mr.name_off.p : nullptr;
		A.gene_names = c->gene_names.p; A.gene_name_off = c->gene_name_off.p;
		A.n_buckets = (unsigned)E.buckets.size();
		A.tables_lds_bytes = tables_bytes;
		A.ablate = c->dev_ablate;
		A.compact = mr.compact ? 1u : 0u;
		A.p1 = mr.p1.p; A.p1_strand = mr.p1_strand.p; A.p1_line = mr.p1_line.p;
		A.p2 = mr.p2.p; A.p2_strand = mr.p2_strand.p; A.p2_line = mr.p2_line.p;
		A.pn_blk_off = mr.pn_blk_off.p; A.pn_nblk = mr.pn_nblk.p; A.pn_se = reinterpret_cast<const int2 *>(mr.pn_se.p);
		A.pn_strand = mr.pn_strand.p; A.pn_line = mr.pn_line.p; A.pn_bucket = mr.pn_bucket.p;
		A.p1_off = mr.p1_off.p; A.p2_off = mr.p2_off.p; A.pn_off = mr.pn_off.p; A.slot_off = mr.slot_off.p;
		A.total_slots = mr.total_slots;
		A.cnt = c->cnt.p + (size_t)m * n_cls; A.bases = c->bases.p + (size_t)m * n_cls;
		A.exc = mr.exc.p + (size_t)set * mr.exc_cap; A.exc_count = c->exc_count.p + 2 * m; A.exc_cap = (unsigned)mr.exc_cap;
		A.dbg = c->dbg.p; A.bar = c->dbg.p + 16 + m;
		A.wg_trace = nullptr;
		const unsigned long long n_pn = mr.pn_strand.n;
		A.n_pn = n_pn;
		const unsigned workers_per_cu = 2;
		A.n_workers = (unsigned)std::min<unsigned long long>((n_pn + COUNT_BLOCK - 1) / COUNT_BLOCK, (unsigned long long)c->n_cu * workers_per_cu);
#ifdef LSQ_DEV
		if (c->dev_ablate & 32768u) A.n_workers = 0;
#endif
		if (c->has_fast) {
			if (c->time_events) HIP_TRY(hipEventRecord(c->evf0[m], st));
			const bool last_streaming = m == M - 1 && !c->has_generic && !c->time_events;
			const dim3 fgrid((unsigned)grid + A.n_workers);
#ifdef LSQ_DEV
			if (c->dev_ablate & 4194304u) {
				if (c->wg_trace.n < 4ull * fgrid.x) { int rc = c->wg_trace.alloc(4ull * fgrid.x); if (rc) return rc; }
				HIP_TRY(hipMemsetAsync(c->wg_trace.p, 0, 4ull * fgrid.x * sizeof(unsigned long long), st));
				c->wg_trace_n = fgrid.x; c->wg_trace_workers = A.n_workers;
				A.wg_trace = c->wg_trace.p;
			}
#endif
			void *kargs[] = {(void *)&A};
			HIP_TRY(hipExtLaunchKernel(mr.compact ? fn_compact : fn_wide, fgrid, dim3(COUNT_BLOCK), kargs, lds_bytes, st, nullptr, last_streaming ? c->ev_counted2[set] : nullptr, 0));
			if (last_streaming) counted_signalled = true;
			if (c->time_events) HIP_TRY(hipEventRecord(c->evf1[m], st));
			c->fast_launched |= 1 << m;
			cleanups.push_back({A, n_pn, m});
		}
		if (c->has_generic) {
			hipLaunchKernelGGL(lsq_count_generic_kernel, dim3((unsigned)grid), dim3(COUNT_BLOCK), generic_tables_bytes, st, A);
			HIP_TRY(hipGetLastError());
		}
	}
	if (c->time_events) HIP_TRY(hipEventRecord(c->ev1, st));
	c->count_timed = c->time_events;
	if (!counted_signalled) HIP_TRY(hipEventRecord(c->ev_counted2[set], st));
	HIP_TRY(hipStreamWaitEvent(st_em, c->ev_counted2[set], 0));
	const unsigned rgrid = std::max(16u, (unsigned)c->n_cu);
	if (c->recount_args.n < 2 * (size_t)LSQ_MAX_METHODS * sizeof(CountArgs)) {
		int rc = c->recount_args.alloc(2 * (size_t)LSQ_MAX_METHODS * sizeof(CountArgs));
		if (rc) return rc;
		c->recount_args_host.assign(2 * (size_t)LSQ_MAX_METHODS * sizeof(CountArgs), 0);
	}
	for (const Cleanup &u : cleanups) {
		const size_t slot = ((size_t)set * LSQ_MAX_METHODS + (size_t)u.m) * sizeof(CountArgs);
		if (memcmp(c->recount_args_host.data() + slot, &u.A, sizeof(CountArgs)) != 0) {
			memcpy(c->recount_args_host.data() + slot, &u.A, sizeof(CountArgs));
			HIP_TRY(hipMemcpyAsync(c->recount_args.p + slot, c->recount_args_host.data() + slot, sizeof(CountArgs), hipMemcpyHostToDevice, st_em));
		}
		const CountArgs *dA = reinterpret_cast<const CountArgs *>(c->recount_args.p + slot);
		hipLaunchKernelGGL(lsq_count_cleanup_kernel, dim3(c->opt_cleanup_grid ? c->opt_cleanup_grid : rgrid), dim3(256), 0, st_em, dA, c->opt_recount ? 1 : 0, u.n_pn,
		                   (const ExcEntry *)u.A.exc, (const unsigned *)u.A.exc_count, u.A.exc_cap);
		HIP_TRY(hipGetLastError());
	}
	return LSQ_OK;
}

}

extern "C" {

int lsq_count_status(lsq_ctx *c, uint32_t *exceptions, uint32_t *recounted) LSQ_API_TRY {
	if (!c) return fail(LSQ_E_ARG, "null context");
	if (!c->counted) return fail(LSQ_E_STATE, "lsq_count must come first");
	HIP_TRY(hipSetDevice(c->device));
	{ int rc = sync_all(c); if (rc) return rc; }
	std::vector<unsigned> h(c->exc_count.n);
	HIP_TRY(hipMemcpy(h.data(), c->exc_count.p, h.size() * sizeof(unsigned), hipMemcpyDeviceToHost));
	note_overflow(c, h);
	for (int m = 0; m < c->E->n_methods; ++m) {
		if (exceptions) exceptions[m] = h[2 * (size_t)m];
		if (recounted) recounted[m] = h[2 * (size_t)m + 1];
	}
	return LSQ_OK;
} LSQ_API_CATCH

int lsq_count_launch_info(lsq_ctx *c, uint32_t *reads_per_look, uint32_t *workgroups_per_cu) LSQ_API_TRY {
	if (!c) return fail(LSQ_E_ARG, "null context");
	if (!c->counted) return fail(LSQ_E_STATE, "lsq_count must come first");
	if (reads_per_look) *reads_per_look = c->last_reads_per_look;
	if (workgroups_per_cu) *workgroups_per_cu = c->last_wg_per_cu;
	return LSQ_OK;
} LSQ_API_CATCH

int lsq_debug_counters(lsq_ctx *c, unsigned long long *out8) LSQ_API_TRY {
	HIP_TRY(hipSetDevice(c->device));
	{ int rc = sync_all(c); if (rc) return rc; }
	HIP_TRY(hipMemcpy(out8, c->dbg.p, 16 * sizeof(unsigned long long), hipMemcpyDeviceToHost));
	std::vector<unsigned> h(c->exc_count.n);
	HIP_TRY(hipMemcpy(h.data(), c->exc_count.p, h.size() * sizeof(unsigned), hipMemcpyDeviceToHost));
	out8[4] = h[0];
	return LSQ_OK;
} LSQ_API_CATCH

int lsq_debug_wg_trace(lsq_ctx *c, unsigned long long *out, unsigned long long cap, unsigned long long *n, unsigned long long *n_workers) LSQ_API_TRY {
	HIP_TRY(hipSetDevice(c->device));
	{ int rc = sync_all(c); if (rc) return rc; }
	const unsigned long long k = std::min<unsigned long long>(cap, c->wg_trace_n);
	if (k) HIP_TRY(hipMemcpy(out, c->wg_trace.p, 4 * k * sizeof(unsigned long long), hipMemcpyDeviceToHost));
	*n = k; *n_workers = c->wg_trace_workers;
	return LSQ_OK;
} LSQ_API_CATCH

int lsq_debug_plan_shares(const unsigned long long *slot_off, const unsigned char *packed, const unsigned long long *n1, const unsigned long long *n2,
                          const unsigned *look1, const unsigned *look2, unsigned long long n_buckets, unsigned long long grid,
                          const double *costs4, int weighted, int snap, unsigned long long *cuts) LSQ_API_TRY {
	if (!slot_off || !packed || !costs4 || !cuts || grid == 0) return fail(LSQ_E_ARG, "null argument");
	lsq::SharePlanCosts pc;
	pc.weighted = weighted != 0; pc.snap = snap != 0;
	pc.two_block = costs4[0]; pc.walk_look = costs4[1]; pc.visit = costs4[2]; pc.taper = costs4[3];
	lsq::plan_share_cuts(slot_off, packed, n1, n2, look1, look2, (size_t)n_buckets, grid, pc, cuts);
	return LSQ_OK;
} LSQ_API_CATCH

int lsq_debug_slot_offsets(lsq_ctx *c, int method, unsigned long long *out, unsigned long long n) LSQ_API_TRY {
	HIP_TRY(hipSetDevice(c->device));
	HIP_TRY(hipStreamSynchronize(c->stream));
	const MethodReads &mr = c->reads[method];
	if (n > mr.slot_off.n) n = mr.slot_off.n;
	HIP_TRY(hipMemcpy(out, mr.slot_off.p, n * sizeof(unsigned long long), hipMemcpyDeviceToHost));
	return LSQ_OK;
} LSQ_API_CATCH

int lsq_debug_offsets(lsq_ctx *c, int method, int which, unsigned long long *out, unsigned long long cap, unsigned long long *n) LSQ_API_TRY {
	HIP_TRY(hipSetDevice(c->device));
	{ int rc = sync_all(c); if (rc) return rc; }
	const MethodReads &mr = c->reads[method];
	if (which == 4 || which == 5) {
		const std::vector<unsigned> &v = which == 4 ? mr.plan_park1 : mr.plan_park2;
		const unsigned long long k = std::min<unsigned long long>(cap, v.size());
		for (unsigned long long i = 0; i < k; ++i) out[i] = v[i];
		*n = k;
		return LSQ_OK;
	}
	const DevBuf<unsigned long long> &src = which == 0 ? mr.slot_off : (which == 1 ? mr.p1_off : (which == 2 ? mr.p2_off : mr.wg_cut));
	const unsigned long long k = std::min<unsigned long long>(cap, src.n);
	if (k) HIP_TRY(hipMemcpy(out, src.p, k * sizeof(unsigned long long), hipMemcpyDeviceToHost));
	*n = k;
	return LSQ_OK;
} LSQ_API_CATCH

}
```

lesseq_amd/csrc/lsq_device.hip:

```cpp
#include "lsq_device.hpp"
#include <chrono>
#include <thread>

namespace lsq {

int upload_strand_ranks(lsq_ctx *c) {
	const auto &names = c->E->strands.names;
	if (names.size() > 256) return fail(LSQ_E_RANGE, "more than 256 distinct strand strings");
	std::vector<int> order(names.size());
	std::iota(order.begin(), order.end(), 0);
	std::sort(order.begin(), order.end(), [&](int a, int b) { return names[a] < names[b]; });
	std::vector<uint8_t> rank(256, 0);
	for (size_t r = 0; r < order.size(); ++r) rank[order[r]] = (uint8_t)r;
	int rc = c->strand_rank.upload(rank.data(), 256, c->stream);
	if (rc) return rc;
	HIP_TRY(hipStreamSynchronize(c->stream));
	return LSQ_OK;
}

static hipError_t wait_for_stream(hipStream_t s) {
	const auto t0 = std::chrono::steady_clock::now();
	for (;;) {
		const hipError_t e = hipStreamQuery(s);
		if (e != hipErrorNotReady) return e;
// ... 737 lines not shown
	float best = 1e30f;
	for (int cfg = 0; cfg < 8; ++cfg) {
		const unsigned grid = (unsigned)c->n_cu * (4u << (cfg & 3));
		for (int it = 0; it < 6; ++it) {
			HIP_TRY(hipEventRecord(a, c->stream));
			if (cfg < 4) hipLaunchKernelGGL(lsq_read_rate_kernel<4>, dim3(grid), dim3(256), 0, c->stream, buf.p, n_words, sink.p);
			else hipLaunchKernelGGL(lsq_read_rate_kernel<8>, dim3(grid), dim3(256), 0, c->stream, buf.p, n_words, sink.p);
			HIP_TRY(hipEventRecord(b, c->stream));
			HIP_TRY(hipEventSynchronize(b));
			float ms = 0;
			HIP_TRY(hipEventElapsedTime(&ms, a, b));
			if (it >= 1) best = std::min(best, ms);
		}
	}
	(void)hipEventDestroy(a); (void)hipEventDestroy(b);
	*gb_per_s = (double)(n_words * 16) / ((double)best * 1e-3) / 1e9;
	return LSQ_OK;
} LSQ_API_CATCH

int lsq_debug_hip_versions(int *compiled, int *runtime) {
	if (compiled) *compiled = HIP_VERSION;
	if (runtime) { int v = 0; if (hipRuntimeGetVersion(&v) != hipSuccess) v = 0; *runtime = v; }
	return LSQ_OK;
}

int lsq_debug_set_em_order(lsq_ctx *c, const uint32_t *order, unsigned n_small_places, unsigned n_places) LSQ_API_TRY {
	HIP_TRY(hipSetDevice(c->device));
	{ int rc = sync_all(c); if (rc) return rc; }
	if (n_small_places > n_places) return fail(LSQ_E_ARG, "more small places than places");
	int rc = c->em_order.upload(order, n_places, c->stream);
	if (rc) return rc;
	HIP_TRY(hipStreamSynchronize(c->stream));
	{
		const size_t np = std::max<size_t>(n_small_places, 1);
		for (int l = 0; l < 2; ++l)
			if (c->em_tail_flag[l].n < np && ((rc = c->em_tail_u32[l].alloc(2 * np)) || (rc = c->em_tail_flag[l].alloc(np)) || (rc = c->em_tail_f64[l].alloc(3 * np)))) return rc;
	}
	c->em_small_places = n_small_places; c->em_places = n_places;
	c->em_order_lane_valid[0] = c->em_order_lane_valid[1] = false;
	c->opt_em_regroup = false;
	return LSQ_OK;
} LSQ_API_CATCH

int lsq_ctx_set_option(lsq_ctx *c, const char *name, double value) LSQ_API_TRY {
	if (!c || !name) return fail(LSQ_E_ARG, "null argument");
	const std::string n(name);
	if (n == "grid_multiplier") {
		if (!(value >= 0 && value <= 64)) return fail(LSQ_E_ARG, "grid_multiplier must lie in 0..64 (0 = automatic)");
		c->opt_grid_mult = value;
		for (auto &r : c->reads) r.wg_grid = 0;
	} else if (n == "exception_capacity") {
		if (!(value >= 0 && value <= 4e9)) return fail(LSQ_E_ARG, "exception_capacity must lie in 0..4e9 (0 = automatic)");
		c->opt_exc_cap = (size_t)value;
	} else if (n == "snap_shares") {
		c->opt_snap_shares = value != 0;
		for (auto &r : c->reads) r.wg_grid = 0;
	} else if (n == "share_weighted" || n == "share_cost_two_block" || n == "share_cost_parked" || n == "share_cost_visit" || n == "share_taper" || n == "share_cost_hot") {
		if (!(value >= 0 && value <= 1e6)) return fail(LSQ_E_ARG, "%s must lie in 0..1e6", name);
		if (n == "share_weighted") c->opt_share_weighted = value != 0;
		else if (n == "share_cost_two_block") c->opt_share_cost_p2 = value;
		else if (n == "share_cost_parked") c->opt_share_cost_park = value;
		else if (n == "share_cost_visit") c->opt_share_cost_visit = value;
		else if (n == "share_cost_hot") c->opt_share_cost_hot = value;
		else c->opt_share_taper = value;
		for (auto &r : c->reads) r.wg_grid = 0;
	} else if (n == "sam_skip_flags") {
		if (!(value >= 0 && value <= 65535)) return fail(LSQ_E_ARG, "sam_skip_flags must lie in 0..65535");
		c->opt_sam_skip_flags = (unsigned)value;
	} else if (n == "sam_min_mapq") {
		if (!(value >= 0 && value <= 256)) return fail(LSQ_E_ARG, "sam_min_mapq must lie in 0..256");
		c->opt_sam_min_mapq = (unsigned)value;
	} else if (n == "bam_verify") {
		if (!(value == 0 || value == 1)) return fail(LSQ_E_ARG, "bam_verify must be 0 or 1");
		c->opt_bam_verify = value == 1;
	} else if (n == "compact_pools") {
		c->opt_compact_pools = value != 0;
	} else if (n == "workgroups_per_cu") {
		if (!(value >= -1 && value <= 32)) return fail(LSQ_E_ARG, "workgroups_per_cu must lie in -1..32 (-1 = automatic, 0 = as many as fit)");
		c->opt_wg_per_cu = (int)value;
		c->occ_lds_bytes = 0;
	} else if (n == "reads_per_look") {
		if (!(value == 0 || value == 4 || value == 8)) return fail(LSQ_E_ARG, "reads_per_look must be 0 (automatic), 4 or 8");
		c->opt_reads_per_look = (int)value;
	} else if (n == "count_streams") {
		{ int rc = sync_all(c); if (rc) return rc; }
		c->opt_two_count_streams = value >= 2;
	} else if (n == "em_flat_min_events") {
		if (!(value >= 0 && value <= 4e9)) return fail(LSQ_E_ARG, "em_flat_min_events must lie in 0..4e9");
		c->opt_em_flat_min = (unsigned)value;
	} else if (n == "em_closed_form") {
		{ int rc = sync_all(c); if (rc) return rc; }
		c->opt_em_closed = value != 0;
	} else if (n == "em_quad_cap") {
		if (value < 0 || value > 1e6) return fail(LSQ_E_ARG, "em_quad_cap out of range");
		c->opt_em_quad_cap = (unsigned)value;
	} else if (n == "em_regroup") {
		c->opt_em_regroup = value != 0;
		c->em_order_lane_valid[0] = c->em_order_lane_valid[1] = false;
	} else if (n == "recount_every_read") {
		c->opt_recount = value != 0;
	} else if (n == "cleanup_workgroups") {
		if (value < 0 || value > 4096) return fail(LSQ_E_ARG, "cleanup_workgroups out of range");
		c->opt_cleanup_grid = (unsigned)value;
	} else if (n == "em_guard_band") {
		return lsq_set_em_guard_band(c, value);
	} else
		return fail(LSQ_E_ARG, "unknown option '%s'", name);
	return LSQ_OK;
} LSQ_API_CATCH

int lsq_set_timing(lsq_ctx *c, int on) LSQ_API_TRY {
	if (!c) return fail(LSQ_E_ARG, "null context");
	c->time_events = on != 0;
	return LSQ_OK;
} LSQ_API_CATCH

int lsq_last_fast_kernel_ms(lsq_ctx *c, float *ms) LSQ_API_TRY {
	if (!c || !ms) return fail(LSQ_E_ARG, "null argument");
	if (!c->counted || !c->count_timed) return fail(LSQ_E_STATE, "the last lsq_count ran without timing (lsq_set_timing)");
	HIP_TRY(hipSetDevice(c->device));
	{ int rc = sync_all(c); if (rc) return rc; }
	*ms = 0;
	for (int m = 0; m < LSQ_MAX_METHODS; ++m) if (c->fast_launched >> m & 1) { float t = 0; HIP_TRY(hipEventElapsedTime(&t, c->evf0[m], c->evf1[m])); *ms += t; }
	return LSQ_OK;
} LSQ_API_CATCH

int lsq_last_timing(lsq_ctx *c, float *count_ms, float *solve_ms) LSQ_API_TRY {
	if (!c) return fail(LSQ_E_ARG, "null context");
	HIP_TRY(hipSetDevice(c->device));
	{ int rc = sync_all(c); if (rc) return rc; }
	if ((count_ms && c->counted && !c->count_timed) || (solve_ms && c->solved && !c->solve_timed))
		return fail(LSQ_E_STATE, "the last lsq_count / lsq_solve ran without timing (lsq_set_timing)");
	if (count_ms) { *count_ms = 0; if (c->counted) HIP_TRY(hipEventElapsedTime(count_ms, c->ev0, c->ev1)); }
	if (solve_ms) { *solve_ms = 0; if (c->solved) HIP_TRY(hipEventElapsedTime(solve_ms, c->ev2, c->ev3)); }
	return LSQ_OK;
} LSQ_API_CATCH

}
```

lesseq_amd/csrc/lsq_device.hpp:

```cpp
#pragma once
#include <hip/hip_runtime.h>

#include <algorithm>
#include <cmath>
#include <cstring>
#include <memory>
#include <numeric>
#include <string>
#include <thread>
#include <type_traits>
#include <vector>

#include "lsq_internal.hpp"

using namespace lsq;

#define HIP_TRY(expr)                                                                          \
	do {                                                                                       \
		hipError_t _e = (expr);                                                                \
		if (_e != hipSuccess) return fail(LSQ_E_DEVICE, "%s: %s", #expr, hipGetErrorString(_e)); \
	} while (0)


#ifndef LSQ_P1_PAD
#define LSQ_P1_PAD 8
#endif
#ifndef LSQ_P2_PAD
#define LSQ_P2_PAD 4
#endif
constexpr unsigned P2_GROUP_PAD = LSQ_P2_PAD;
constexpr unsigned P1_GROUP_PAD = LSQ_P1_PAD;
constexpr int LSQ_INGEST_STAGES = 7;
constexpr int LSQ_INGEST_PASS_MAX = 16;
constexpr int EM_LANES = 4;

namespace lsq {

constexpr unsigned COMPACT_OFF_BITS = 22, COMPACT_OFF_MASK = (1u << COMPACT_OFF_BITS) - 1u, COMPACT_MAX_LEN = 1u << 10;
constexpr int COMPACT_BIAS = 1 << 21;
__host__ __device__ inline bool compact_block_fits(long long off, long long len) { return off >= 0 && off <= (long long)COMPACT_OFF_MASK && len > 0 && len < (long long)COMPACT_MAX_LEN; }

struct ExcEntry {
	unsigned long long slot;
	unsigned bucket;
	unsigned ev_pool_scan;
};

template <class T>
struct DevBuf {
	T *p = nullptr;
	size_t n = 0;
	~DevBuf() { if (p) (void)hipFree(p); }
	int alloc(size_t count) {
		if (p) { (void)hipFree(p); p = nullptr; }
		n = count;
		HIP_TRY(hipMalloc((void **)&p, std::max<size_t>(count, 1) * sizeof(T)));
		return LSQ_OK;
	}
	int upload(const T *src, size_t count, hipStream_t st) {
		int rc = alloc(count);
		if (rc) return rc;
		if (count) HIP_TRY(hipMemcpyAsync(p, src, count * sizeof(T), hipMemcpyHostToDevice, st));
		return LSQ_OK;
	}
};

template <class T>
struct DevView { T *p = nullptr; size_t n = 0; };

struct RouteChrom {
	unsigned loc_first, loc_nb;
	int loc_base;
	unsigned cov0, cov1, clu0, clu1;
	unsigned pad;
};
static_assert(sizeof(RouteChrom) == 32, "RouteChrom is staged in LDS as two 16-byte words");

struct VisitRec {
	BucketDesc d;
	unsigned long long bs, be;
	unsigned long long p1o, p1n, p2o, p2n;
	unsigned b, next;
	unsigned pad[2];
};
static_assert(sizeof(VisitRec) == 128, "VisitRec is read as 32 dwords");
struct WgPlan {
	unsigned long long s_begin, s_end;
	VisitRec first;
};
static_assert(sizeof(WgPlan) == 144, "WgPlan layout");

struct IngestPass {
	const char *name = nullptr;
	hipEvent_t ev[2] = {nullptr, nullptr};
	unsigned long long bytes = 0;
	float ms = 0;
	bool clocked = false;
};

struct MethodReads {
	DevBuf<ExcEntry> exc;
	size_t exc_cap = 0;
	bool present = false;
	uint64_t n_retained = 0, n_retained_blocks = 0, total_slots = 0;
	uint64_t lib_report[5] = {0, 0, 0, 0, 0};
	DevBuf<int32_t> p1, p2, pn_se;
	bool compact = false;
	uint64_t n1_reads = 0, n2_reads = 0;
	DevBuf<uint8_t> p1_strand, p2_strand, pn_strand;
	DevBuf<uint32_t> p1_line, p2_line, pn_line, pn_blk_off, pn_nblk, pn_bucket;
	DevBuf<unsigned long long> p1_off, p2_off, pn_off, pnb_off, slot_off;
	double skew = 1.0;
	bool named = false;
	DevBuf<char> names;
	DevBuf<unsigned long long> name_off;
	DevBuf<unsigned> wg_first;
	DevBuf<unsigned long long> wg_cut;
	DevBuf<WgPlan> wg_plan;
	std::vector<VisitRec> visits_host;
	std::vector<unsigned long long> slot_off_host;
	DevBuf<VisitRec> visits;
	std::vector<unsigned long long> plan_n1, plan_n2;
	std::vector<unsigned long long> plan_seg_x;
	std::vector<unsigned char> plan_seg_kind;
	std::vector<unsigned> plan_seg_looks, plan_seg_first;
	std::vector<unsigned> plan_park1, plan_park2;
	std::vector<unsigned> next_packed_host;
	unsigned long long wg_grid = 0;
};

}

struct lsq_ctx {
	std::thread lanes_thread;
	int lanes_status = 0;
	std::string lanes_error;
	int device = 0;
	int n_cu = 256;
	hipStream_t stream = nullptr;
	hipStream_t stream_em = nullptr;
	hipStream_t stream_em2[2] = {nullptr, nullptr};
	hipStream_t stream_count2[2] = {nullptr, nullptr};
	bool opt_two_count_streams = true;
	int opt_wg_per_cu = -1;
	hipEvent_t ev_counted2[2] = {nullptr, nullptr}, ev_mark2[2] = {nullptr, nullptr};
	bool mark_recorded2[2] = {false, false};
	int flip = 0;
	size_t counters_per_set = 0;
	hipEvent_t ev0 = nullptr, ev1 = nullptr, ev2 = nullptr, ev3 = nullptr;
	hipEvent_t evt0 = nullptr, evt1 = nullptr;
	hipEvent_t evf0[LSQ_MAX_METHODS] = {}, evf1[LSQ_MAX_METHODS] = {};
	int fast_launched = 0;
	int occ_p1w = 0;
	int opt_reads_per_look = 0;
	unsigned last_reads_per_look = 4, last_wg_per_cu = 0;
	unsigned occ_lds_bytes = 0; int occ_blocks = 0;
	bool time_events = false;
	bool count_timed = false, solve_timed = false;
	lsq_events *E = nullptr;
	DevBuf<BucketDesc> buckets;
	DevBuf<uint8_t> images, strand_rank, dK;
	DevBuf<TieRec> ties;
	DevBuf<uint32_t> cls_base, iso_base, em_order, gene_name_off;
	DevBuf<char> gene_names;
	DevBuf<uint32_t> pack_cls, pack_iso, pack_ev;
	DevBuf<uint32_t> em_order_lane[2];
	DevBuf<uint32_t> em_split;
	bool em_order_lane_valid[2] = {false, false};
	unsigned em_regroup_age[2] = {0, 0};
	bool opt_em_regroup = true;
	bool opt_em_closed = false;
	unsigned opt_em_quad_cap = 0;
	DevBuf<uint32_t> em_tail_count, em_tail_u32[2];
	DevBuf<uint8_t> em_tail_flag[2];
	DevBuf<double> em_tail_f64[2];
	unsigned opt_em_flat_min = 16384;
	unsigned em_places = 0;
	unsigned em_small_places = 0;
	DevBuf<double> G, theta2[2], logll2[2];
	DevBuf<uint32_t> iters2[2];
	DevBuf<uint8_t> flags2[2];
	DevView<double> theta, logll;
	DevView<uint32_t> iters;
	DevView<uint8_t> flags;
	DevBuf<uint32_t> fim_start_base, fim_mat_base, fim_starts;
	DevBuf<double> fim, fim_var;
	size_t fim_starts_total = 0, fim_mat_total = 0;
	bool fim_uploaded = false, fim_done = false;
	DevBuf<unsigned long long> counters;
	DevView<unsigned long long> cnt, bases, dbg;
	DevBuf<unsigned long long> wg_trace;
	unsigned long long wg_trace_n = 0, wg_trace_workers = 0;
	DevView<unsigned> exc_count;
	DevBuf<RouteChrom> route_chrom;
	DevBuf<int2> cov;
	DevBuf<int4> clu;
	DevBuf<uint2> loc;
	unsigned loc_shift = 10;
	DevBuf<unsigned> bin_base;
	size_t n_fine = 0;
	DevBuf<unsigned> cell_base;
	size_t n_cell_groups = 0;
	DevBuf<unsigned long long> jg_keys;
	DevBuf<unsigned> jg_base, jgroup_base;
	size_t n_junction_groups = 0;
	unsigned n_chrom_tables = 0;
	double opt_grid_mult = 0;
	size_t opt_exc_cap = 0;
	bool opt_compact_pools = true;
	bool opt_recount = false;
	unsigned opt_cleanup_grid = 0;
	bool overflow_logged[LSQ_MAX_METHODS] = {};
	bool opt_snap_shares = true;
	bool opt_share_weighted = true;
	double opt_share_cost_p2 = 4.3;
	double opt_share_cost_park = 9.0;
	double opt_share_cost_visit = 7000.0;
	double opt_share_cost_hot = 0.5;
	double opt_share_taper = 0;
	unsigned dev_ablate = 0;
	DevBuf<unsigned char> recount_args;
	std::vector<unsigned char> recount_args_host;
	MethodReads reads[LSQ_MAX_METHODS];
	bool counted = false, solved = false;
	bool counts_external = false;
	double em_band = 1E-11;
	bool has_fast = false, has_generic = false, has_host = false;
	uint64_t host_genes = 0, host_reads = 0;
	std::map<size_t, std::vector<unsigned short>> host_seq;
	float count_ms = 0, solve_ms = 0;
	float mrf_h2d_ms = 0, mrf_parse_ms = 0;
	unsigned parse_tiles_handed = 0, parse_lines_listed = 0, parse_all_slow = 0;
	unsigned opt_sam_skip_flags = 0x904u, opt_sam_min_mapq = 0u;
	bool opt_bam_verify = false;
	unsigned sam_lines_listed = 0, sam_all_slow = 0;
	unsigned long long bam_blocks = 0, bam_blocks_repaired = 0;
	unsigned char *pin_buf[2] = {nullptr, nullptr};
	hipEvent_t pin_ev[2] = {nullptr, nullptr};
// ... 28 lines not shown
```

lesseq_amd/csrc/lsq_ingest.hip:

```cpp
#include "lsq_ingest.hpp"
#include "lsq_text.hpp"

namespace {

struct IngestRaw {
	unsigned long long n_reads;
	const unsigned long long *blk_off;
	const unsigned *line_no;
	const int *blk_start, *blk_end;
	const unsigned short *blk_chrom;
	const unsigned char *blk_strand;
};

#ifndef LSQ_RAW_WAVES
#define LSQ_RAW_WAVES 8
#endif
template <bool STRANDED, class... Lib>
__global__ void __launch_bounds__(256) __attribute__((amdgpu_waves_per_eu(LSQ_RAW_WAVES))) lsq_route_raw_kernel(RouteTables T, IngestRaw R, RouteOut O, Lib... lib_arg) {
	__shared__ RouteChrom chrom_lds[ROUTE_CHROM_LDS];
	const RouteChrom *chroms = route_stage_chroms(T, chrom_lds);
	const unsigned long long gsz = (unsigned long long)gridDim.x * blockDim.x;
	LocProbe P;
	P.chrom = -1; P.bin = 0;
	if constexpr (!STRANDED) {
// ... 308 lines not shown
		unsigned g[4]; uint4 v[4], x[4]; bool on[4];
#pragma unroll
		for (int u = 0; u < 4; ++u) {
			const unsigned r = r0 + 256u * (unsigned)u;
			on[u] = r < pc.z;
			g[u] = on[u] ? fine[r] - gbase : 0u;
			if (!pool) { v[u] = on[u] ? A.part1[first + r] : make_uint4(0, 0, 0, 0); x[u] = v[u]; }
			else { v[u] = on[u] ? A.part2[2ull * (first + r)] : make_uint4(0, 0, 0, 0); x[u] = on[u] ? A.part2[2ull * (first + r) + 1] : make_uint4(0, 0, 0, 0); }
		}
#pragma unroll
		for (int u = 0; u < 4; ++u) {
			if (!on[u]) continue;
			const unsigned long long w = off0 + goff[g[u]] + atomicAdd(&cur[g[u]], 1u);
			if (!pool) {
				const int2 rec = make_int2((int)v[u].x, (int)v[u].y);
				if (A.compact) pool_store<true>(A.p1, w, rec, base); else pool_store<false>(A.p1, w, rec, base);
				A.p1_strand[w] = (unsigned char)v[u].w; A.p1_line[w] = v[u].z;
			} else {
				const int4 rec = make_int4((int)v[u].x, (int)v[u].y, (int)v[u].z, (int)v[u].w);
				if (A.compact) pool_store<true>(A.p2, w, rec, base); else pool_store<false>(A.p2, w, rec, base);
				A.p2_strand[w] = (unsigned char)x[u].y; A.p2_line[w] = x[u].x;
			}
		}
	}
}

struct NbOut {
	const uint4 *ent; const int2 *blk; unsigned long long n_ent;
	const unsigned long long *pn_off, *pnb_off;
	unsigned *curn, *curnb;
	unsigned *pn_blk_off, *pn_nblk, *pn_line, *pn_bucket; unsigned char *pn_strand; int2 *pn_se;
	const unsigned *line_no; unsigned long long first_line;
};
__global__ void __launch_bounds__(256) lsq_ingest_nblock_kernel(NbOut O) {
	const unsigned long long gsz = (unsigned long long)gridDim.x * blockDim.x;
	for (unsigned long long t = (unsigned long long)blockIdx.x * blockDim.x + threadIdx.x; t < O.n_ent; t += gsz) {
		const uint4 en = O.ent[t];
		const unsigned i = en.x, b = en.y, n = en.z & 0xFFu, strand = en.z >> 8;
		const unsigned long long w = O.pn_off[b] + atomicAdd(&O.curn[b], 1u);
		const unsigned long long bo = O.pnb_off[b] + atomicAdd(&O.curnb[b], n);
		O.pn_blk_off[w] = (unsigned)bo; O.pn_nblk[w] = n; O.pn_bucket[w] = b;
		O.pn_strand[w] = (unsigned char)strand; O.pn_line[w] = O.line_no ? O.line_no[i] : (unsigned)(O.first_line + i);
		for (unsigned q = 0; q < n; ++q) O.pn_se[bo + q] = O.blk[(unsigned long long)en.w + q];
	}
}

__global__ void __launch_bounds__(256) lsq_ingest_pad_kernel(const BucketDesc *buckets, const unsigned *cell_base, const unsigned *jgroup_base, unsigned n_buckets,
                                                             unsigned n_groups1, unsigned n_groups2, const unsigned *cnt1, const unsigned long long *off1,
                                                             const unsigned *cnt2, const unsigned long long *off2, const unsigned char *images,
                                                             void *p1, void *p2, unsigned compact, unsigned char *p1_strand, unsigned *p1_line,
                                                             unsigned char *p2_strand, unsigned *p2_line) {
	for (unsigned t = blockIdx.x * blockDim.x + threadIdx.x; t < n_groups1 + n_groups2; t += gridDim.x * blockDim.x) {
		const bool one = t < n_groups1;
		const unsigned g = one ? t : t - n_groups1;
		const unsigned n = one ? cnt1[g] : cnt2[g], gp = one ? P1_GROUP_PAD : P2_GROUP_PAD, pad = ((n + gp - 1u) & ~(gp - 1u)) - n;
		if (!pad) continue;
		const unsigned *gbase = one ? cell_base : jgroup_base;
		unsigned lo_b = 0, hi_b = n_buckets;
		while (hi_b - lo_b > 1) { const unsigned mid = (lo_b + hi_b) >> 1; if (gbase[mid] <= g) lo_b = mid; else hi_b = mid; }
		const BucketDesc &d = buckets[lo_b];
		const int base = d.lo - lsq::COMPACT_BIAS;
		if (!one) {
			for (unsigned q = 0; q < pad; ++q) {
				const unsigned long long w = off2[g] + n + q;
				if (compact) reinterpret_cast<uint2 *>(p2)[w] = make_uint2((unsigned)lsq::COMPACT_BIAS, 0u);
				else reinterpret_cast<int4 *>(p2)[w] = make_int4(d.lo, d.lo, d.lo, d.lo);
				p2_strand[w] = 0; p2_line[w] = 0;
			}
			continue;
		}
		const unsigned cell = g - cell_base[lo_b];
		int at = d.lo;
		if (d.kind == 1u && cell < (d.iso_off & 0xFFFFu)) at = reinterpret_cast<const lsq::Cell *>(images + d.img_off + d.seg_off)[cell].lo;
		if (compact && !lsq::compact_block_fits((long long)at - base, 1)) at = base;
		for (unsigned q = 0; q < pad; ++q) {
			const unsigned long long w = off1[g] + n + q;
			if (compact) reinterpret_cast<unsigned *>(p1)[w] = (unsigned)(at - base);
			else reinterpret_cast<int2 *>(p1)[w] = make_int2(at, at);
			p1_strand[w] = 0; p1_line[w] = 0;
		}
	}
}

static const char *const INGEST_STAGE_NAMES[LSQ_INGEST_STAGES] = {
	"newline_count", "route", "partition_count", "partition_scatter", "group_classify", "group_offsets", "group_place"};

void stages_collect(lsq_ctx *c) {
	for (int k = 0; k < c->ing_n; ++k) {
		IngestPass &p = c->ing_pass[k];
		float ms = 0;
		if (p.clocked && p.ev[0] && p.ev[1] && hipEventElapsedTime(&ms, p.ev[0], p.ev[1]) == hipSuccess) p.ms = ms;
	}
	(void)hipGetLastError();
}

}

unsigned lsq::route_lib(const lsq_ctx *c) {
	const lsq_events &E = *c->E;
	return E.stranded() ? route_lib_word(E.library == LSQ_LIBRARY_REVERSE, (unsigned)E.strand_plus, (unsigned)E.strand_minus) : 0u;
}
RouteTables lsq::route_tables(lsq_ctx *c) {
	RouteTables T{};
	T.chrom = c->route_chrom.p; T.cov = c->cov.p; T.clu = c->clu.p; T.loc = c->loc.p; T.loc_shift = c->loc_shift; T.n_chrom = c->n_chrom_tables;
	return T;
}

int lsq::ingest_device(lsq_ctx *c, int method, Front &F) {
	HostStopwatch SW;
	const lsq_events &E = *c->E;
	MethodReads &mr = c->reads[method];
	mr.present = false;
	const unsigned B = (unsigned)E.buckets.size();
	const unsigned long long n = F.n;
	if (B >= ROUTE_NO_BUCKET) return fail(LSQ_E_RANGE, "more than 2^22 buckets");
	if (n > 0xFFFFFFF0ull) return fail(LSQ_E_RANGE, "more than 2^32 reads in one file");
	hipStream_t st = c->stream;
	int rc;
	if ((rc = ensure_lanes(c))) return rc;
	HIP_TRY(hipStreamSynchronize(c->stream_em2[0]));
	HIP_TRY(hipStreamSynchronize(c->stream_em2[1]));
	HIP_TRY(hipStreamSynchronize(c->stream_count2[0]));
	HIP_TRY(hipStreamSynchronize(c->stream_count2[1]));
	const size_t FC = c->n_cell_groups;
	const size_t FJ = c->n_junction_groups;
	const size_t n_cnt = 10 * (size_t)B + 3 * (FC + FJ);
	const size_t n_tot = 8 + ROUTE_LIB_WORD0 + (E.stranded() ? 8 * (size_t)ROUTE_LIB_SLOTS : 0);
	std::vector<unsigned long long> lib_places(E.stranded() ? 8 * (size_t)ROUTE_LIB_SLOTS : 0);
	DevBuf<unsigned> d_key, d_cnt, d_fine1, d_fine2;
	DevBuf<int4> d_rec;
	DevBuf<unsigned long long> d_tot, d_part_off1, d_part_off2, d_piece_off, d_off1, d_off2;
	DevBuf<uint4> d_nb_ent, d_part1, d_part2, d_pieces;
	DevBuf<int2> d_nb_blk;
	ScanScratch SS;
	if ((rc = d_key.alloc(n)) || (rc = d_rec.alloc(n)) || (rc = d_cnt.alloc(n_cnt)) || (rc = d_tot.alloc(n_tot)) || (rc = d_part_off1.alloc(B + 1)) || (rc = d_part_off2.alloc(B + 1)) ||
	    (rc = d_piece_off.alloc(2 * (size_t)B + 1)) || (rc = d_off1.alloc(FC + 1)) || (rc = d_off2.alloc(FJ + 1)) || (rc = SS.reserve(std::max<size_t>(std::max(FC, FJ), 2 * (size_t)B)))) return rc;
	unsigned *part_cnt = d_cnt.p, *part_cur = part_cnt + 2 * (size_t)B, *piece_cnt = part_cur + 2 * (size_t)B;
	unsigned *cntn = piece_cnt + 2 * (size_t)B, *cntnb = cntn + B, *curn = cntnb + B, *curnb = curn + B;
	unsigned *cnt1 = curnb + B, *cnt2 = cnt1 + FC, *cur1 = cnt2 + FJ, *cur2 = cur1 + FC, *park1 = cur2 + FJ, *park2 = park1 + FC;
	if ((rc = mr.p1_off.alloc(B + 1)) || (rc = mr.p2_off.alloc(B + 1)) || (rc = mr.pn_off.alloc(B + 1)) || (rc = mr.pnb_off.alloc(B + 1)) || (rc = mr.slot_off.alloc(B + 1))) return rc;
	const RouteTables T = route_tables(c);
	const size_t part_lds = 8 * (size_t)B;
	const bool part_in_lds = part_lds <= 128 * 1024 && getenv("LSQ_PART_NO_LDS") == nullptr;
	size_t img_max = 16, jg_max = 0, groups_max = 1;
	for (unsigned b = 0; b < B; ++b) {
		const BucketDesc &d = E.buckets[b];
		const size_t n_cells = d.kind == 1u ? (d.iso_off & 0xFFFFu) : 0u, n_jg = E.jg_base[b + 1] - E.jg_base[b];
		if (d.kind == 1u) img_max = std::max<size_t>(img_max, (d.img_bytes + 15u) & ~15u);
		jg_max = std::max(jg_max, n_jg);
		groups_max = std::max(groups_max, n_jg + n_cells + 1);
	}
	const size_t keys_lds = (8 * jg_max + 15) & ~(size_t)15, group_lds = img_max + keys_lds + 8 * groups_max, place_lds = 8 * groups_max;
	if (group_lds > 160 * 1024) return fail(LSQ_E_UNSUPPORTED, "a bucket's tables and group counters exceed the CU's LDS");
	if (part_in_lds && part_lds > 48 * 1024) {
		HIP_TRY(hipFuncSetAttribute((const void *)lsq_part_hist_kernel<true>, hipFuncAttributeMaxDynamicSharedMemorySize, (int)part_lds));
		HIP_TRY(hipFuncSetAttribute((const void *)lsq_part_scatter_kernel<true>, hipFuncAttributeMaxDynamicSharedMemorySize, (int)part_lds));
	}
	if (group_lds > 48 * 1024) HIP_TRY(hipFuncSetAttribute((const void *)lsq_group_classify_kernel, hipFuncAttributeMaxDynamicSharedMemorySize, (int)group_lds));
	if (place_lds > 48 * 1024) HIP_TRY(hipFuncSetAttribute((const void *)lsq_group_place_kernel, hipFuncAttributeMaxDynamicSharedMemorySize, (int)place_lds));
	const unsigned part_grid = (unsigned)std::max<unsigned long long>(1, std::min<unsigned long long>(n / 131072ull, 2ull * (unsigned)c->n_cu));
	SW.mark("ingest: allocations");
	if (!c->ing_n) (void)stage_entry(c, INGEST_STAGE_NAMES[0]);
	(void)stage_entry(c, F.stage);
	for (int s = 2; s < LSQ_INGEST_STAGES; ++s) (void)stage_entry(c, INGEST_STAGE_NAMES[s]);
	c->ing_reported = c->ing_n;

// ... 16 lines not shown
		}
		{
			StageClock k(c, st, "partition_count");
			if (part_in_lds) hipLaunchKernelGGL(lsq_part_hist_kernel<true>, dim3(part_grid), dim3(PART_WG), part_lds, st, (const unsigned *)d_key.p, n, B, part_cnt, d_tot.p);
			else hipLaunchKernelGGL(lsq_part_hist_kernel<false>, dim3(part_grid), dim3(PART_WG), 0, st, (const unsigned *)d_key.p, n, B, part_cnt, d_tot.p);
			HIP_TRY(hipGetLastError());
			if ((rc = device_scan<1>(SS, part_cnt, B, d_part_off1.p, st)) || (rc = device_scan<1>(SS, part_cnt + B, B, d_part_off2.p, st)) ||
			    (rc = device_scan<1>(SS, cntn, B, mr.pn_off.p, st)) || (rc = device_scan<1>(SS, cntnb, B, mr.pnb_off.p, st))) return rc;
			hipLaunchKernelGGL(lsq_piece_count_kernel, dim3(2 * B / 256 + 1), dim3(256), 0, st, (const unsigned *)part_cnt, 2 * B, piece_cnt);
			HIP_TRY(hipGetLastError());
			if ((rc = device_scan<1>(SS, piece_cnt, 2ull * B, d_piece_off.p, st))) return rc;
			k.end(4ull * n);
		}
		HIP_TRY(hipMemcpyAsync(tot, d_tot.p, 8 * 8, hipMemcpyDeviceToHost, st));
		HIP_TRY(hipMemcpyAsync(nb_tot, d_tot.p + 8, 8 * 8, hipMemcpyDeviceToHost, st));
		if (!lib_places.empty()) HIP_TRY(hipMemcpyAsync(lib_places.data(), d_tot.p + 8 + ROUTE_LIB_WORD0, lib_places.size() * 8, hipMemcpyDeviceToHost, st));
		HIP_TRY(hipMemcpyAsync(&sums[0], d_part_off1.p + B, 8, hipMemcpyDeviceToHost, st));
		HIP_TRY(hipMemcpyAsync(&sums[1], d_part_off2.p + B, 8, hipMemcpyDeviceToHost, st));
		HIP_TRY(hipMemcpyAsync(&sums[2], d_piece_off.p + 2 * (size_t)B, 8, hipMemcpyDeviceToHost, st));
		HIP_TRY(hipMemcpyAsync(&sums[3], mr.pn_off.p + B, 8, hipMemcpyDeviceToHost, st));
		HIP_TRY(hipMemcpyAsync(&sums[4], mr.pnb_off.p + B, 8, hipMemcpyDeviceToHost, st));
		HIP_TRY(hipStreamSynchronize(st));
		SW.mark("ingest: route + partition counts");
		if (F.settle && (rc = F.settle(st))) { if (rc == LSQ_RETRY) continue; return rc; }
		const bool go_wide = compact && tot[3] * 16 > tot[4] + tot[5] + tot[3];
		const bool list_short = nb_tot[0] > nb_cap || nb_tot[1] > nbb_cap;
		if (go_wide || list_short) {
			if (go_wide) compact = 0;
			if (list_short) { nb_cap = std::max(nb_cap, nb_tot[0]); nbb_cap = std::max(nbb_cap, nb_tot[1]); }
			continue;
		}
		break;
	}
	if (nb_tot[2]) return fail(LSQ_E_RANGE, "a read covers 2^18 or more bases or keeps more than %d separate blocks: outside the device tables' range", INGEST_MAX_BLOCKS);
	if (sums[4] > 0xFFFFFFF0ull) return fail(LSQ_E_RANGE, "too many blocks in multi-block reads");
	const size_t n1p = (size_t)sums[0], n2p = (size_t)sums[1], n_pieces = (size_t)sums[2], nn = (size_t)sums[3], nnb = (size_t)sums[4];
	if (n_pieces > 0x7FFFFFFFull) return fail(LSQ_E_RANGE, "too many partition pieces");
	if ((rc = d_part1.alloc(n1p)) || (rc = d_part2.alloc(2 * n2p)) || (rc = d_fine1.alloc(n1p)) || (rc = d_fine2.alloc(n2p)) || (rc = d_pieces.alloc(n_pieces))) return rc;
	SW.mark("ingest: partition buffers");
	{
		StageClock k(c, st, "partition_scatter");
		PartArgs A{};
		A.key = d_key.p; A.rec = d_rec.p; A.n = n; A.B = B; A.off1 = d_part_off1.p; A.off2 = d_part_off2.p; A.cursor = part_cur;
		A.part1 = d_part1.p; A.part2 = d_part2.p; A.line_no = F.line_no; A.first_line = F.first_line;
		if (n1p + n2p) {
			if (part_in_lds) hipLaunchKernelGGL(lsq_part_scatter_kernel<true>, dim3(part_grid), dim3(PART_WG), part_lds, st, A);
			else hipLaunchKernelGGL(lsq_part_scatter_kernel<false>, dim3(part_grid), dim3(PART_WG), 0, st, A);
		}
		hipLaunchKernelGGL(lsq_piece_expand_kernel, dim3(2 * B / 256 + 1), dim3(256), 0, st, (const unsigned *)part_cnt, (const unsigned long long *)d_piece_off.p, 2 * B, d_pieces.p);
		HIP_TRY(hipGetLastError());
		k.end(8ull * n + 16ull * (n1p + n2p) + 16ull * n1p + 32ull * n2p);
	}
	GroupArgs GA{};
	GA.pieces = d_pieces.p; GA.off1 = d_part_off1.p; GA.off2 = d_part_off2.p; GA.part1 = d_part1.p; GA.part2 = d_part2.p;
	GA.fine1 = d_fine1.p; GA.fine2 = d_fine2.p; GA.cnt1 = cnt1; GA.cnt2 = cnt2; GA.park1 = park1; GA.park2 = park2;
	if (n_pieces) {
		StageClock k(c, st, "group_classify");
		GroupTables GT{};
		GT.buckets = c->buckets.p; GT.images = c->images.p; GT.cell_base = c->cell_base.p; GT.jg_keys = c->jg_keys.p; GT.jg_base = c->jg_base.p; GT.jgroup_base = c->jgroup_base.p;
		GT.B = B; GT.lds_img = (unsigned)img_max; GT.lds_keys = (unsigned)keys_lds;
		hipLaunchKernelGGL(lsq_group_classify_kernel, dim3((unsigned)n_pieces), dim3(256), group_lds, st, GT, GA);
		HIP_TRY(hipGetLastError());
		k.end(16ull * n1p + 32ull * n2p + 4ull * (n1p + n2p));
	}
	unsigned long long psum[2] = {0, 0};
	{
		StageClock k(c, st, "group_offsets");
		if ((rc = device_scan<P1_GROUP_PAD>(SS, cnt1, FC, d_off1.p, st)) || (rc = device_scan<P2_GROUP_PAD>(SS, cnt2, FJ, d_off2.p, st))) return rc;
		hipLaunchKernelGGL(lsq_ingest_offsets_kernel, dim3(B / 256 + 1), dim3(256), 0, st, c->cell_base.p, c->jgroup_base.p, B, d_off1.p, d_off2.p, mr.pn_off.p,
		                   mr.p1_off.p, mr.p2_off.p, mr.slot_off.p);
		HIP_TRY(hipGetLastError());
		k.end(12ull * (FC + FJ));
	}
	SW.mark("ingest: partition + group launches");
	HIP_TRY(hipMemcpyAsync(&psum[0], mr.p1_off.p + B, 8, hipMemcpyDeviceToHost, st));
	HIP_TRY(hipMemcpyAsync(&psum[1], mr.p2_off.p + B, 8, hipMemcpyDeviceToHost, st));
	HIP_TRY(hipStreamSynchronize(st));
	SW.mark("ingest: partition + groups");
	const size_t n1 = (size_t)psum[0], n2 = (size_t)psum[1];
	mr.compact = compact != 0;
	mr.n1_reads = tot[4]; mr.n2_reads = tot[5];
	if ((rc = mr.p1.alloc(mr.compact ? ((n1 + 3) & ~(size_t)3) : 2 * n1)) || (rc = mr.p1_strand.alloc(n1)) || (rc = mr.p1_line.alloc(n1))) return rc;
	if ((rc = mr.p2.alloc(mr.compact ? 2 * ((n2 + 1) & ~(size_t)1) : 4 * n2)) || (rc = mr.p2_strand.alloc(n2)) || (rc = mr.p2_line.alloc(n2))) return rc;
	if ((rc = mr.pn_se.alloc(2 * nnb)) || (rc = mr.pn_blk_off.alloc(nn)) || (rc = mr.pn_nblk.alloc(nn)) || (rc = mr.pn_strand.alloc(nn)) ||
	    (rc = mr.pn_line.alloc(nn)) || (rc = mr.pn_bucket.alloc(nn))) return rc;
	{
		StageClock k(c, st, "group_place");
		if (n_pieces) {
			PlaceArgs P{};
			P.pieces = d_pieces.p; P.part_off1 = d_part_off1.p; P.part_off2 = d_part_off2.p; P.part1 = d_part1.p; P.part2 = d_part2.p;
			P.fine1 = d_fine1.p; P.fine2 = d_fine2.p; P.off1 = d_off1.p; P.off2 = d_off2.p; P.cur1 = cur1; P.cur2 = cur2;
			P.buckets = c->buckets.p; P.cell_base = c->cell_base.p; P.jg_base = c->jg_base.p; P.jgroup_base = c->jgroup_base.p; P.B = B; P.compact = compact;
			P.p1 = mr.p1.p; P.p1_strand = mr.p1_strand.p; P.p1_line = mr.p1_line.p; P.p2 = mr.p2.p; P.p2_strand = mr.p2_strand.p; P.p2_line = mr.p2_line.p;
			hipLaunchKernelGGL(lsq_group_place_kernel, dim3((unsigned)n_pieces), dim3(256), place_lds, st, P);
		}
		if (FC + FJ) {
			const unsigned pgrid = (unsigned)std::min<size_t>((FC + FJ) / 256 + 1, (size_t)c->n_cu * 8);
			hipLaunchKernelGGL(lsq_ingest_pad_kernel, dim3(pgrid), dim3(256), 0, st, c->buckets.p, c->cell_base.p, c->jgroup_base.p, B, (unsigned)FC, (unsigned)FJ,
			                   (const unsigned *)cnt1, (const unsigned long long *)d_off1.p, (const unsigned *)cnt2, (const unsigned long long *)d_off2.p, c->images.p,
			                   (void *)mr.p1.p, (void *)mr.p2.p, compact, mr.p1_strand.p, mr.p1_line.p, mr.p2_strand.p, mr.p2_line.p);
		}
		if (nn) {
			NbOut N{};
			N.ent = d_nb_ent.p; N.blk = d_nb_blk.p; N.n_ent = nb_tot[0]; N.pn_off = mr.pn_off.p; N.pnb_off = mr.pnb_off.p; N.curn = curn; N.curnb = curnb;
			N.pn_blk_off = mr.pn_blk_off.p; N.pn_nblk = mr.pn_nblk.p; N.pn_line = mr.pn_line.p; N.pn_bucket = mr.pn_bucket.p; N.pn_strand = mr.pn_strand.p;
			N.pn_se = reinterpret_cast<int2 *>(mr.pn_se.p); N.line_no = F.line_no; N.first_line = F.first_line;
			const unsigned ngrid = (unsigned)std::min<unsigned long long>((nb_tot[0] + 255) / 256, (unsigned long long)c->n_cu * 16);
			hipLaunchKernelGGL(lsq_ingest_nblock_kernel, dim3(ngrid), dim3(256), 0, st, N);
		}
		HIP_TRY(hipGetLastError());
		k.end(16ull * n1p + 32ull * n2p + 4ull * (n1p + n2p) + (mr.compact ? 4ull : 8ull) * (n1 + 2 * n2) + 5ull * (n1 + n2));
	}
	{
		size_t want = std::max<size_t>(65536, (n1 + n2) / 4);
		if (c->opt_exc_cap) want = c->opt_exc_cap;
		if (mr.exc_cap != want) {
			if ((rc = mr.exc.alloc(2 * want))) return rc;
			mr.exc_cap = want;
		}
	}
	if ((rc = upload_strand_ranks(c))) return rc;
	mr.n_retained = tot[0];
	for (int q = 0; q < 5; ++q) {
		mr.lib_report[q] = 0;
		for (size_t k = 0; k < lib_places.size(); k += 8) mr.lib_report[q] += lib_places[k + q];
	}
	mr.n_retained_blocks = tot[1] + nb_tot[1];
	mr.total_slots = n1 + n2 + nn;
	mr.wg_grid = 0;
	{
		std::vector<unsigned long long> so(B + 1, 0), o1(B + 1, 0), o2(B + 1, 0), f1(FC + 1, 0), f2(FJ + 1, 0);
		std::vector<unsigned> park(FC + FJ + 1, 0);
		HIP_TRY(hipMemcpyAsync(so.data(), mr.slot_off.p, (B + 1) * sizeof(unsigned long long), hipMemcpyDeviceToHost, st));
		HIP_TRY(hipMemcpyAsync(o1.data(), mr.p1_off.p, (B + 1) * sizeof(unsigned long long), hipMemcpyDeviceToHost, st));
		HIP_TRY(hipMemcpyAsync(o2.data(), mr.p2_off.p, (B + 1) * sizeof(unsigned long long), hipMemcpyDeviceToHost, st));
		HIP_TRY(hipMemcpyAsync(f1.data(), d_off1.p, (FC + 1) * sizeof(unsigned long long), hipMemcpyDeviceToHost, st));
		HIP_TRY(hipMemcpyAsync(f2.data(), d_off2.p, (FJ + 1) * sizeof(unsigned long long), hipMemcpyDeviceToHost, st));
		if (FC + FJ) HIP_TRY(hipMemcpyAsync(park.data(), park1, (FC + FJ) * sizeof(unsigned), hipMemcpyDeviceToHost, st));
		HIP_TRY(hipStreamSynchronize(st));
		SW.mark("ingest: place + read-back");
		stages_collect(c);
		unsigned long long mx = 0;
		for (unsigned b = 0; b < B; ++b) mx = std::max(mx, so[b + 1] - so[b]);
		mr.slot_off_host = so;
		mr.skew = (B && mr.total_slots) ? (double)mx * (double)B / (double)mr.total_slots : 1.0;
		{
			mr.plan_n1.resize(B); mr.plan_n2.resize(B); mr.plan_park1.assign(B, 0); mr.plan_park2.assign(B, 0);
			mr.plan_seg_x.clear(); mr.plan_seg_kind.clear(); mr.plan_seg_looks.clear(); mr.plan_seg_first.assign(B + 1, 0);
			size_t g1 = 0, g2 = 0;
			for (unsigned b = 0; b < B; ++b) {
				const unsigned n_cg = (E.buckets[b].kind == 1 ? (E.buckets[b].iso_off & 0xFFFFu) : 0u) + 1u, n_jg = (E.jg_base[b + 1] - E.jg_base[b]) + n_cg;
				const unsigned long long n1 = o1[b + 1] - o1[b], n2 = o2[b + 1] - o2[b], ns = so[b + 1] - so[b];
				mr.plan_n1[b] = n1; mr.plan_n2[b] = n2;
				mr.plan_seg_first[b] = (unsigned)mr.plan_seg_kind.size();
				const bool visited = E.buckets[b].kind == 1u && ns != 0;
				if (visited) {
					for (unsigned q = 0; q < n_cg && g1 + q < FC; ++q) {
						const unsigned long long a = f1[g1 + q], e = f1[g1 + q + 1];
						mr.plan_park1[b] += park[g1 + q];
						if (e > a) { mr.plan_seg_x.push_back(so[b] + (a - o1[b])); mr.plan_seg_kind.push_back(0); mr.plan_seg_looks.push_back(park[g1 + q]); }
					}
					for (unsigned q = 0; q < n_jg && g2 + q < FJ; ++q) {
						const unsigned long long a = f2[g2 + q], e = f2[g2 + q + 1];
						mr.plan_park2[b] += park[FC + g2 + q];
						if (e > a) { mr.plan_seg_x.push_back(so[b] + n1 + (a - o2[b])); mr.plan_seg_kind.push_back(1); mr.plan_seg_looks.push_back(park[FC + g2 + q]); }
					}
					if (ns > n1 + n2) { mr.plan_seg_x.push_back(so[b] + n1 + n2); mr.plan_seg_kind.push_back(2); mr.plan_seg_looks.push_back(0); }
				} else if (ns) { mr.plan_seg_x.push_back(so[b]); mr.plan_seg_kind.push_back(2); mr.plan_seg_looks.push_back(0); }
				g1 += n_cg; g2 += n_jg;
			}
			mr.plan_seg_first[B] = (unsigned)mr.plan_seg_kind.size();
			mr.plan_seg_x.push_back(B ? so[B] : 0);
		}
		std::vector<VisitRec> vis(B + 1);
		mr.next_packed_host.assign(B + 1, B);
		memset(vis.data(), 0, vis.size() * sizeof(VisitRec));
		unsigned next = B;
		for (unsigned b = B; b-- > 0;) {
			VisitRec &v = vis[b];
			v.d = E.buckets[b];
			v.bs = so[b]; v.be = so[b + 1];
			v.p1o = o1[b]; v.p1n = o1[b + 1] - o1[b]; v.p2o = o2[b]; v.p2n = o2[b + 1] - o2[b];
			v.b = b; v.next = next;
			if (E.buckets[b].kind == 1u && so[b + 1] > so[b]) next = b;
			mr.next_packed_host[b] = next;
		}
		vis[B].b = B; vis[B].next = B; vis[B].bs = vis[B].be = mr.total_slots;
		if ((rc = mr.visits.upload(vis.data(), vis.size(), st))) return rc;
		mr.visits_host = vis;
		HIP_TRY(hipStreamSynchronize(st));
	}
	mr.present = true;
	c->counted = c->solved = false;
	SW.mark("ingest: plan, visit records");
	return LSQ_OK;
}

namespace {

void front_of_raw(lsq_ctx *c, const IngestRaw &Rw, unsigned long long n_blocks, Front &F) {
	F.n = Rw.n_reads; F.line_no = Rw.line_no; F.first_line = 0;
	F.in_bytes = 12ull * Rw.n_reads + 11ull * n_blocks;
	F.launch = [c, Rw](const RouteTables &T, const RouteOut &O, hipStream_t st) -> int {
		const unsigned igrid = (unsigned)std::min<unsigned long long>((Rw.n_reads + 255) / 256 + 1, (unsigned long long)c->n_cu * 16);
		if (c->E->stranded()) hipLaunchKernelGGL((lsq_route_raw_kernel<true, unsigned>), dim3(igrid), dim3(256), 0, st, T, Rw, O, route_lib(c));
		else hipLaunchKernelGGL(lsq_route_raw_kernel<false>, dim3(igrid), dim3(256), 0, st, T, Rw, O);
		HIP_TRY(hipGetLastError());
		return LSQ_OK;
	};
}

}

extern "C" {

int lsq_reads_upload(lsq_ctx *c, int method, const lsq_reads *R) LSQ_API_TRY {
	if (!c || !R) return fail(LSQ_E_ARG, "null argument");
	if (!c->E) return fail(LSQ_E_STATE, "lsq_events_upload must come first");
	if (method < 0 || method >= c->E->n_methods) return fail(LSQ_E_ARG, "method %d out of range", method);
	HIP_TRY(hipSetDevice(c->device));
	const uint64_t n = R->n_reads, nblk = R->n_blocks;
	hipStream_t st = c->stream;
	int rc;
	HostStopwatch SW;
	DevBuf<unsigned long long> d_blk_off;
	DevBuf<unsigned> d_line;
	DevBuf<int> d_bs, d_be;
	DevBuf<unsigned short> d_bc;
	DevBuf<unsigned char> d_bst;
	const unsigned long long zero_off = 0;
	auto up = [&](auto &buf, const auto *src, size_t count, const char *what) -> int {
		typedef typename std::remove_reference<decltype(*buf.p)>::type E;
		const size_t bytes = count * sizeof(E);
		if (bytes < (64ull << 20)) return buf.upload(src, count, st);
		int r2 = buf.alloc(count);
		if (r2) return r2;
		const unsigned char *s8 = reinterpret_cast<const unsigned char *>(src);
		return pinned_pipeline(c, reinterpret_cast<unsigned char *>(buf.p), bytes, [s8](unsigned char *dst, size_t off, size_t nby) { memcpy(dst, s8 + off, nby); return true; }, what);
	};
	if ((rc = up(d_blk_off, n ? (const unsigned long long *)R->blk_off : &zero_off, n + 1, "block offsets"))) return rc;
	if ((rc = up(d_line, R->line_no, n, "line numbers"))) return rc;
	if ((rc = up(d_bs, R->blk_start, nblk, "block starts"))) return rc;
	if ((rc = up(d_be, R->blk_end, nblk, "block ends"))) return rc;
	if ((rc = up(d_bc, R->blk_chrom, nblk, "block chromosomes"))) return rc;
	if ((rc = up(d_bst, R->blk_strand, nblk, "block strands"))) return rc;
	IngestRaw Rw{};
	Rw.n_reads = n; Rw.blk_off = d_blk_off.p; Rw.line_no = d_line.p; Rw.blk_start = d_bs.p; Rw.blk_end = d_be.p;
	Rw.blk_chrom = d_bc.p; Rw.blk_strand = d_bst.p;
	SW.mark("upload: allocations, copies queued");
	if (SW.on) { HIP_TRY(hipStreamSynchronize(st)); SW.mark("upload: copies done"); }
	stages_reset(c, false);
	Front F;
	front_of_raw(c, Rw, nblk, F);
	if ((rc = ingest_device(c, method, F))) return rc;
	MethodReads &mr = c->reads[method];
	mr.named = R->named;
	if (R->named) {
		if ((rc = mr.names.upload(R->name_blob.data(), R->name_blob.size(), st))) return rc;
		if ((rc = mr.name_off.upload((const unsigned long long *)R->name_off.data(), R->name_off.size(), st))) return rc;
		HIP_TRY(hipStreamSynchronize(st));
	}
	return LSQ_OK;
} LSQ_API_CATCH

int lsq_ingest_stage_count(void) { return LSQ_INGEST_STAGES; }
const char *lsq_ingest_stage_name(int stage) { return stage >= 0 && stage < LSQ_INGEST_STAGES ? INGEST_STAGE_NAMES[stage] : nullptr; }
int lsq_last_ingest_stage_count(const lsq_ctx *c) { return c && c->ing_reported ? c->ing_reported : LSQ_INGEST_STAGES; }
const char *lsq_last_ingest_stage_name(const lsq_ctx *c, int stage) {
	if (stage < 0 || stage >= lsq_last_ingest_stage_count(c)) return nullptr;
	return c && c->ing_reported ? c->ing_pass[stage].name : lsq_ingest_stage_name(stage);
}
int lsq_last_ingest_stages(const lsq_ctx *c, float *ms, uint64_t *bytes, int capacity) LSQ_API_TRY {
	if (!c) return fail(LSQ_E_ARG, "null context");
	for (int k = 0; k < lsq_last_ingest_stage_count(c) && k < capacity; ++k) {
		if (ms) ms[k] = c->ing_reported ? c->ing_pass[k].ms : 0.0f;
		if (bytes) bytes[k] = c->ing_reported ? c->ing_pass[k].bytes : 0;
	}
	return LSQ_OK;
} LSQ_API_CATCH

uint64_t lsq_reads_retained(const lsq_ctx *c, int method) { return (c && method >= 0 && method < LSQ_MAX_METHODS) ? c->reads[method].n_retained : 0; }
uint64_t lsq_reads_pooled(const lsq_ctx *c, int method) {
	if (!c || method < 0 || method >= LSQ_MAX_METHODS) return 0;
	const MethodReads &mr = c->reads[method];
	return mr.n1_reads + mr.n2_reads + mr.pn_line.n;
}
uint64_t lsq_reads_pooled_blocks(const lsq_ctx *c, int method) {
	if (!c || method < 0 || method >= LSQ_MAX_METHODS) return 0;
	const MethodReads &mr = c->reads[method];
	return mr.n1_reads + 2 * mr.n2_reads + mr.pn_se.n / 2;
}
int lsq_last_library_report(const lsq_ctx *c, int method, uint64_t out[5]) LSQ_API_TRY {
	if (!c || !out || method < 0 || method >= LSQ_MAX_METHODS) return fail(LSQ_E_ARG, "bad context or method");
	if (!c->E || !c->E->stranded()) return fail(LSQ_E_STATE, "the events of this context are unstranded: there is no library report");
	if (!c->reads[method].present) return fail(LSQ_E_STATE, "no reads uploaded for method %d", method);
	for (int q = 0; q < 5; ++q) out[q] = c->reads[method].lib_report[q];
	return LSQ_OK;
} LSQ_API_CATCH
uint64_t lsq_reads_retained_blocks(const lsq_ctx *c, int method) { return (c && method >= 0 && method < LSQ_MAX_METHODS) ? c->reads[method].n_retained_blocks : 0; }

int lsq_reads_pool_format(const lsq_ctx *c, int method, int *compact, uint64_t *pool_bytes, uint64_t *pool_reads) LSQ_API_TRY {
	if (!c || method < 0 || method >= LSQ_MAX_METHODS) return fail(LSQ_E_ARG, "bad context or method");
	const MethodReads &mr = c->reads[method];
	if (!mr.present) return fail(LSQ_E_STATE, "no reads uploaded for method %d", method);
	if (compact) *compact = mr.compact ? 1 : 0;
	if (pool_bytes) *pool_bytes = 4ull * (mr.p1.n + mr.p2.n + mr.pn_se.n);
	if (pool_reads) { pool_reads[0] = mr.n1_reads; pool_reads[1] = mr.n2_reads; pool_reads[2] = mr.pn_line.n; }
	return LSQ_OK;
} LSQ_API_CATCH

}
```

Baseline: 744.4 billion reads/s.

## Add dense delta-encoded pool1 stream with per-group anchors for the count kernel

At ingest time, groups of eight compact single-block reads are re-encoded as a 16-byte word of eight 16-bit offsets plus an 8-byte anchor holding the minimum start, the minimum length and precomputed length surpluses against the cell thresholds. A new dense variant of the fast count kernel streams this 24-byte-per-group format instead of the 32-byte compact pool. It decides whole groups against the event ends by comparing offsets to thresholds, falling back to the original records for mixed or non-dense groups. The kernel is selected by default when few groups are non-dense. This reduces bytes read per read but adds an ingest pass, extra device buffers and more branching in the hot loop.

```diff
diff --git a/include/lesseq_hip.h b/include/lesseq_hip.h
--- a/include/lesseq_hip.h
+++ b/include/lesseq_hip.h
@@ -144,6 +144,7 @@
 int lsq_count(lsq_ctx *c);
 int lsq_count_status(lsq_ctx *c, uint32_t *exceptions, uint32_t *recounted);
 int lsq_count_launch_info(lsq_ctx *c, uint32_t *reads_per_look, uint32_t *workgroups_per_cu);
+int lsq_reads_dense_info(lsq_ctx *c, int method, uint64_t *groups, uint64_t *not_dense, uint64_t *mixed, int *used, uint64_t *stream_bytes);
 int lsq_host_evaluated(const lsq_ctx *c, uint64_t *n_genes, uint64_t *n_reads);
 int lsq_ctx_set_option(lsq_ctx *c, const char *name, double value);
 
diff --git a/include/lesseq_hip_dev.h b/include/lesseq_hip_dev.h
--- a/include/lesseq_hip_dev.h
+++ b/include/lesseq_hip_dev.h
@@ -16,6 +16,7 @@
                           const unsigned *look1, const unsigned *look2, unsigned long long n_buckets, unsigned long long grid,
                           const double *costs4, int weighted, int snap, unsigned long long *cuts);
 int lsq_debug_offsets(lsq_ctx *c, int method, int which, unsigned long long *out, unsigned long long cap, unsigned long long *n);
+int lsq_debug_dense_stream(lsq_ctx *c, int method, uint32_t *anchors, uint16_t *offsets, uint32_t *records, unsigned long long cap, unsigned long long *n);
 
 int lsq_debug_set_em_order(lsq_ctx *c, const uint32_t *order, unsigned n_small_places, unsigned n_places);
 
diff --git a/lesseq_amd/_lib.py b/lesseq_amd/_lib.py
--- a/lesseq_amd/_lib.py
+++ b/lesseq_amd/_lib.py
@@ -138,6 +138,9 @@
 _sig("lsq_results_solve", C.c_int, vp, P(C.c_double), P(C.c_double), P(u32), P(u8))
 _sig("lsq_count_status", C.c_int, vp, P(u32), P(u32))
 _sig("lsq_count_launch_info", C.c_int, vp, P(u32), P(u32))
+if hasattr(lib, "lsq_reads_dense_info"):
+    _sig("lsq_reads_dense_info", C.c_int, vp, C.c_int, P(u64), P(u64), P(u64), P(C.c_int), P(u64))
+    _sig("lsq_debug_dense_stream", C.c_int, vp, C.c_int, P(u32), P(u16), P(u32), C.c_ulonglong, P(C.c_ulonglong))
 _sig("lsq_host_evaluated", C.c_int, vp, P(u64), P(u64))
 _sig("lsq_counts_device_words", u64, vp)
 _sig("lsq_counts_export_device", C.c_int, vp, vp)
diff --git a/lesseq_amd/api.py b/lesseq_amd/api.py
--- a/lesseq_amd/api.py
+++ b/lesseq_amd/api.py
@@ -433,6 +433,23 @@
         check(lib.lsq_count_launch_info(self.h, C.byref(a), C.byref(b)))
         return int(a.value), int(b.value)
 
+    def dense_info(self, method):
+        g, nd, mx, used = u64(0), u64(0), u64(0), C.c_int(0)
+        check(lib.lsq_reads_dense_info(self.h, method, C.byref(g), C.byref(nd), C.byref(mx), C.byref(used), None))
+        return int(g.value), int(nd.value), int(mx.value), bool(used.value)
+
+    def dense_stream_bytes(self, method):
+        b = u64(0)
+        check(lib.lsq_reads_dense_info(self.h, method, None, None, None, None, C.byref(b)))
+        return int(b.value)
+
+    def dense_stream(self, method):
+        G = self.dense_info(method)[0]
+        a, o, r = np.zeros((max(G, 1), 2), np.uint32), np.zeros((max(G, 1), 8), np.uint16), np.zeros((max(G, 1), 8), np.uint32)
+        n = C.c_ulonglong(0)
+        check(lib.lsq_debug_dense_stream(self.h, method, _ptr(a, u32), _ptr(o, u16), _ptr(r, u32), G, C.byref(n)))
+        return a[:n.value], o[:n.value], r[:n.value]
+
     def set_em_guard_band(self, band):
         check(lib.lsq_set_em_guard_band(self.h, float(band)))
 
diff --git a/lesseq_amd/csrc/lsq_count.hip b/lesseq_amd/csrc/lsq_count.hip
--- a/lesseq_amd/csrc/lsq_count.hip
+++ b/lesseq_amd/csrc/lsq_count.hip
@@ -27,6 +27,7 @@
 	unsigned ablate;
 	unsigned tables_lds_bytes;
 	const void *p1; const unsigned char *p1_strand; const unsigned *p1_line;
+	const uint2 *p1a; const uint4 *p1d;
 	const void *p2; const unsigned char *p2_strand; const unsigned *p2_line;
 	unsigned compact;
 	const unsigned *pn_blk_off; const unsigned *pn_nblk; const int2 *pn_se; const unsigned char *pn_strand; const unsigned *pn_line; const unsigned *pn_bucket;
@@ -661,6 +662,37 @@
 }
 
 
+template <int NR, class InRange>
+__device__ inline void park_pool1_records(FastCtx &C, Ring<1> &R, const CountArgs &A, const unsigned (&rec)[NR], const InRange &in_range, const unsigned lane,
+                                          const bool has, const bool both, const uint4 cx, const int e1, const int e2, const int base) {
+#pragma unroll
+	for (int h = 0; h < NR; h += 2) {
+		uint4 en[2];
+		unsigned open = 0;
+#pragma unroll
+		for (int j = h; j < h + 2; ++j) {
+			const unsigned len = rec[j] >> lsq::COMPACT_OFF_BITS;
+			const int so = (int)(rec[j] & lsq::COMPACT_OFF_MASK), e = so + (int)len;
+			unsigned rel;
+			const bool in = in_range(j, rel);
+			const bool gone_near = both && (cx.z & CELLX_NEAR_NO_ABUT) != 0u && e > e1 && 50 * (e - e1) >= (int)len;
+			const bool gone_far = both && (cx.z & CELLX_FAR_NO_ABUT) != 0u && e > e2 && 50 * (e - e2) >= (int)len;
+			const bool done_near = e <= e1 || gone_near, done_far = e <= e2 || gone_far;
+			const bool op = in && len != 0u && !(both ? (done_near && done_far) : e <= e2);
+			open |= op ? 1u << (j - h) : 0u;
+			const unsigned hint = !has ? PARK_EVENT_UNKNOWN : (!both ? (cx.w | PARK_ONE_EVENT) :
+			                      (done_far ? (cx.w | PARK_ONE_EVENT) : (done_near ? ((cx.z & 0xFFFFu) | PARK_ONE_EVENT) : PARK_EVENT_UNKNOWN)));
+			en[j - h] = make_uint4((unsigned)(so + base), (unsigned)(so + base) + len, hint, rel);
+			if (ABL(A, 256u) && op) { atomicAdd(&A.dbg[5 + (has ? (both ? 2 : 1) : 0)], 1ull); atomicAdd(&A.dbg[0], 1ull); }
+		}
+		R.push2(open, lane, en[0], en[1]);
+		if (R.live() >= 64u) {
+			if (!ABL(A, 32u)) walk_parked<1, false>(C, R, false, base);
+			else R.head = R.tail;
+		}
+	}
+}
+
 template <int NR>
 __device__ inline void stream_pool1_compact(FastCtx &C, const uint4 *bins, const uint4 *cells, const uint4 *cellx, const unsigned n_cells, const BucketDesc &d,
                                             const CountArgs &A, uint4 *queue, const void *pool, const unsigned long long g0, const unsigned long long g1) {
@@ -744,34 +776,133 @@
 			const bool any_open = __any(lane_open);
 			if (lane == 0) { atomicAdd(&A.dbg[12], 1ull); atomicAdd(&A.dbg[11], any_open ? 1ull : 0ull); }
 		}
-		if (__any(lane_open) && !ABL(A, 17u | 524288u)) {
-#pragma unroll
-			for (int h = 0; h < NR; h += 2) {
-				uint4 en[2];
-				unsigned open = 0;
-#pragma unroll
-				for (int j = h; j < h + 2; ++j) {
-					const unsigned len = rec[j] >> lsq::COMPACT_OFF_BITS;
-					const int so = (int)(rec[j] & lsq::COMPACT_OFF_MASK), e = so + (int)len;
-					const unsigned idx = t + lane * (unsigned)NR + (unsigned)j, rel = idx - first_rel;
-					const bool in = idx < n && rel < n_rel;
-					const bool gone_near = both && (cx.z & CELLX_NEAR_NO_ABUT) != 0u && e > e1 && 50 * (e - e1) >= (int)len;
-					const bool gone_far = both && (cx.z & CELLX_FAR_NO_ABUT) != 0u && e > e2 && 50 * (e - e2) >= (int)len;
-					const bool done_near = e <= e1 || gone_near, done_far = e <= e2 || gone_far;
-					const bool op = in && len != 0u && !(both ? (done_near && done_far) : e <= e2);
-					open |= op ? 1u << (j - h) : 0u;
-					const unsigned hint = !has ? PARK_EVENT_UNKNOWN : (!both ? (cx.w | PARK_ONE_EVENT) :
-					                      (done_far ? (cx.w | PARK_ONE_EVENT) : (done_near ? ((cx.z & 0xFFFFu) | PARK_ONE_EVENT) : PARK_EVENT_UNKNOWN)));
-					en[j - h] = make_uint4((unsigned)(so + base), (unsigned)(so + base) + len, hint, rel);
-					if (ABL(A, 256u) && op) { atomicAdd(&A.dbg[5 + (has ? (both ? 2 : 1) : 0)], 1ull); atomicAdd(&A.dbg[0], 1ull); }
+		if (__any(lane_open) && !ABL(A, 17u | 524288u))
+			park_pool1_records<NR>(C, R, A, rec, [&](const int j, unsigned &rel) { const unsigned idx = t + lane * (unsigned)NR + (unsigned)j; rel = idx - first_rel; return idx < n && rel < n_rel; },
+			                       lane, has, both, cx, e1, e2, base);
+	}
+	if (R.live() && !ABL(A, 32u)) walk_parked<1, false>(C, R, true, base);
+}
+
+__device__ inline void stream_pool1_dense(FastCtx &C, const uint4 *bins, const uint4 *cells, const uint4 *cellx, const unsigned n_cells, const BucketDesc &d,
+                                          const CountArgs &A, uint4 *queue, const unsigned long long g0, const unsigned long long g1) {
+	constexpr int NR = 8;
+	static_assert((unsigned)NR == P1_GROUP_PAD, "a lane takes one whole group of the pool per step");
+	constexpr unsigned TILE = 64u * NR;
+	typedef unsigned u32x2 __attribute__((ext_vector_type(2)));
+	typedef const u32x2 __attribute__((address_space(1))) *global_pairs;
+	C.pool = 0u;
+	C.slot0 = g0;
+	global_words src_d = (global_words)A.p1d, src_p = (global_words)A.p1;
+	global_pairs src_a = (global_pairs)A.p1a;
+	const unsigned lane = threadIdx.x & 63u, wave = (unsigned)__builtin_amdgcn_readfirstlane((int)(threadIdx.x >> 6));
+	const unsigned long long R0 = g0 & ~(unsigned long long)(NR - 1), G0 = R0 >> 3;
+	const unsigned n = (unsigned)(g1 - R0), first_rel = (unsigned)(g0 - R0);
+	const unsigned last_group = (n - 1u) >> 3;
+	const int base = d.lo - lsq::COMPACT_BIAS;
+	uint4 nxt_d; uint2 nxt_a;
+	auto fetch = [&](const unsigned t) {
+		const unsigned g = min((t >> 3) + lane, last_group);
+		const u32x4 v = src_d[G0 + g];
+		const u32x2 w = src_a[G0 + g];
+		nxt_d = make_uint4(v.x, v.y, v.z, v.w);
+		nxt_a = make_uint2(w.x, w.y);
+	};
+	Ring<1> R;
+	R.q = queue;
+	const unsigned t_begin = min(wave * TILE, n);
+	if (t_begin < n) fetch(t_begin);
+	for (unsigned t = t_begin; t < n; t += WAVES * TILE) {
+		const unsigned dw[4] = {nxt_d.x, nxt_d.y, nxt_d.z, nxt_d.w};
+		const unsigned anchor = nxt_a.x, surplus = nxt_a.y;
+		if (t + WAVES * TILE < n) fetch(t + WAVES * TILE);
+		if (ABL(A, 512u)) {
+			asm volatile("" ::"v"(dw[0]), "v"(dw[1]), "v"(dw[2]), "v"(dw[3]), "v"(anchor), "v"(surplus));
+			continue;
+		}
+		const unsigned aoff = anchor & lsq::COMPACT_OFF_MASK, len_g = anchor >> lsq::COMPACT_OFF_BITS;
+		const int p0 = (int)aoff + base;
+		const int rel0 = p0 - d.lo;
+		const unsigned bin = rel0 <= 0 ? 0u : ((unsigned)rel0 >> d.shift);
+		const uint4 br = bins[min(bin, d.n_bins - 1u)];
+		unsigned ci = (br.x & 0xFFFFu) + (unsigned)(p0 >= (int)br.y) + (unsigned)(p0 >= (int)br.z) + (unsigned)(p0 >= (int)br.w);
+		if (__any(p0 >= (int)br.w) && !ABL(A, 65536u)) {
+			while (ci + 1u < n_cells && p0 >= (int)cells[ci + 1u].x) ++ci;
+		}
+		const unsigned cc = min(ci, n_cells - 1u);
+		const uint4 cw = cells[cc];
+		const uint4 cx = cellx[cc];
+		const bool has = ci < n_cells && (int)cw.x <= p0 && p0 < (int)cw.y && !ABL(A, 8u);
+		const bool both = has && (cx.z & CELLX_BOTH) != 0;
+		const int e1 = has ? (int)cw.z - base : -1, e2 = has ? (int)cw.w - base : -1;
+		const unsigned s1 = cx.x & 0xFFFFu, s2 = cx.x >> 16;
+		const bool interior = t + TILE <= n && t >= first_rel;
+		const bool step_dense = interior && !__any(len_g == 0u);
+		bool lane_open = false;
+		if (step_dense) {
+			const int t1 = min(e1 - (int)aoff - (int)len_g, (int)lsq::DENSE_MAX_OFF), t2 = min(e2 - (int)aoff - (int)len_g, (int)lsq::DENSE_MAX_OFF);
+			unsigned nN = 0, nA = 0, nL = 0;
+			auto decide = [&](auto one_threshold) {
+#pragma unroll
+				for (int j = 0; j < NR; ++j) {
+					const int off = (int)((j & 1) ? dw[j >> 1] >> 16 : dw[j >> 1] & 0xFFFFu);
+					nN += (unsigned)(off <= (int)lsq::DENSE_MAX_OFF);
+					nA += (unsigned)(off <= t1);
+					if (!decltype(one_threshold)::value) nL += (unsigned)(off <= t2);
 				}
-				R.push2(open, lane, en[0], en[1]);
-				if (R.live() >= 64u) {
-					if (!ABL(A, 32u)) walk_parked<1, false>(C, R, false, base);
-					else R.head = R.tail;
-				}
-			}
-		}
+				if (decltype(one_threshold)::value) nL = nA;
+			};
+			const bool one = __all(e1 == e2) && !ABL(A, 8388608u);
+			if (one) decide(std::true_type{}); else decide(std::false_type{});
+			if (!ABL(A, (1u | 16384u))) {
+				const unsigned bA = nA * len_g + (surplus & 0x7FFFu), bL = one ? bA : nL * len_g + (surplus >> 16);
+				const unsigned n2 = both ? nL : nL - nA, b2 = both ? bL : bL - bA;
+				if (nA && s1 != CELL_NONE) atomicAdd(&C.hist[s1], ((unsigned long long)nA << 40) | (unsigned long long)bA);
+				if (n2 && s2 != CELL_NONE) atomicAdd(&C.hist[s2], ((unsigned long long)n2 << 40) | (unsigned long long)b2);
+			} else asm volatile("" ::"v"(nA), "v"(nL));
+			lane_open = nN != (both ? nA : nL);
+			if (ABL(A, 256u)) {
+				const bool any_open = __any(lane_open);
+				if (lane == 0) { atomicAdd(&A.dbg[12], 1ull); atomicAdd(&A.dbg[11], any_open ? 1ull : 0ull); }
+			}
+			if (!__any(lane_open)) continue;
+		}
+		unsigned rec[NR];
+#pragma unroll
+		for (int j = 0; j < NR; ++j) {
+			const unsigned off = (j & 1) ? dw[j >> 1] >> 16 : dw[j >> 1] & 0xFFFFu;
+			rec[j] = off == lsq::DENSE_PAD ? aoff : ((aoff + off) | (len_g << lsq::COMPACT_OFF_BITS));
+		}
+		if (len_g == 0u || ((surplus & lsq::DENSE_MIXED) != 0u && (lane_open || !step_dense))) {
+			const unsigned long long w = 2ull * (G0 + min((t >> 3) + lane, last_group));
+			const u32x4 v0 = src_p[w], v1 = src_p[w + 1ull];
+			rec[0] = v0.x; rec[1] = v0.y; rec[2] = v0.z; rec[3] = v0.w; rec[4] = v1.x; rec[5] = v1.y; rec[6] = v1.z; rec[7] = v1.w;
+		}
+		const int j_lo = (int)first_rel - (int)(t + lane * (unsigned)NR), j_hi = (int)n - (int)(t + lane * (unsigned)NR);
+		if (!step_dense) {
+			unsigned accN = 0, accA = 0, accL = 0;
+#pragma unroll
+			for (int j = 0; j < NR; ++j) {
+				const unsigned len = rec[j] >> lsq::COMPACT_OFF_BITS;
+				const int e = (int)(rec[j] & lsq::COMPACT_OFF_MASK) + (int)len;
+				unsigned p = len | (min(len, 1u) << 24);
+				p = (j >= j_lo && j < j_hi) ? p : 0u;
+				accN += p;
+				accA += e <= e1 ? p : 0u;
+				accL += e <= e2 ? p : 0u;
+			}
+			if (!ABL(A, (1u | 16384u))) {
+				const unsigned acc2 = both ? accL : accL - accA;
+				if (accA && s1 != CELL_NONE) atomicAdd(&C.hist[s1], ((unsigned long long)(accA >> 24) << 40) | (accA & 0xFFFFFFu));
+				if (acc2 && s2 != CELL_NONE) atomicAdd(&C.hist[s2], ((unsigned long long)(acc2 >> 24) << 40) | (acc2 & 0xFFFFFFu));
+			} else asm volatile("" ::"v"(accA), "v"(accL));
+			lane_open = (accN >> 24) != ((both ? accA : accL) >> 24);
+			if (ABL(A, 256u)) {
+				const bool any_open = __any(lane_open);
+				if (lane == 0) { atomicAdd(&A.dbg[12], 1ull); atomicAdd(&A.dbg[11], any_open ? 1ull : 0ull); }
+			}
+		}
+		if (__any(lane_open) && !ABL(A, 17u | 524288u))
+			park_pool1_records<NR>(C, R, A, rec, [&](const int j, unsigned &rel) { rel = (unsigned)(j - j_lo); return j >= j_lo && j < j_hi; }, lane, has, both, cx, e1, e2, base);
 	}
 	if (R.live() && !ABL(A, 32u)) walk_parked<1, false>(C, R, true, base);
 }
@@ -1005,8 +1136,9 @@
 #ifndef LSQ_FAST_WAVES
 #define LSQ_FAST_WAVES 6
 #endif
-template <bool COMPACT, int P1W>
+template <bool COMPACT, int P1W, bool DENSE = false>
 __global__ void __launch_bounds__(COUNT_BLOCK, P1W == 4 ? 5 : LSQ_FAST_WAVES) lsq_count_fast_kernel(CountArgs A) {
+	static_assert(!DENSE || (COMPACT && P1W == 4), "the dense stream belongs to the compact pool's eight-reads loop");
 	extern __shared__ __align__(16) unsigned char lds[];
 	const unsigned tid = threadIdx.x;
 	struct Trace {
@@ -1063,7 +1195,8 @@
 		const unsigned long long l0 = (s_begin > bs ? s_begin : bs) - bs;
 		const unsigned long long l1 = (s_end < be ? s_end : be) - bs;
 		if (l0 < n1 && !ABL(A, 1024u)) {
-			if constexpr (COMPACT) stream_pool1_compact<2 * P1W>(C, bins, cells, cellx, n_cells, d, A, wave_queue, A.p1, p1o + l0, p1o + (l1 < n1 ? l1 : n1));
+			if constexpr (DENSE) stream_pool1_dense(C, bins, cells, cellx, n_cells, d, A, wave_queue, p1o + l0, p1o + (l1 < n1 ? l1 : n1));
+			else if constexpr (COMPACT) stream_pool1_compact<2 * P1W>(C, bins, cells, cellx, n_cells, d, A, wave_queue, A.p1, p1o + l0, p1o + (l1 < n1 ? l1 : n1));
 			else stream_pool_wide<2>(C, bins, cells, cellx, n_cells, d, A, wave_queue, reinterpret_cast<const uint4 *>(A.p1), p1o + l0, p1o + (l1 < n1 ? l1 : n1));
 		}
 		if (l1 > n1 && l0 < n1 + n2 && !ABL(A, 2048u)) {
@@ -1319,7 +1452,14 @@
 	const void *const fn_wide = (const void *)lsq_count_fast_kernel<false, 2>;
 	const void *const fn_compact = p1w == 4 ? (const void *)lsq_count_fast_kernel<true, 4> : (const void *)lsq_count_fast_kernel<true, 2>;
 	c->last_reads_per_look = 2u * (unsigned)p1w;
+	const void *const fn_dense = (const void *)lsq_count_fast_kernel<true, 4, true>;
+	auto runs_dense = [&](const MethodReads &r) {
+		if (p1w != 4 || !r.compact || !r.dense_groups || c->opt_dense_pool1 == 0) return false;
+		return c->opt_dense_pool1 == 2 || (r.dense_not * 2048 <= r.dense_groups && r.dense_mixed * 4 <= r.dense_groups);
+	};
+	c->last_dense = 0;
 	if (lds_bytes > 64 * 1024) {
+		HIP_TRY(hipFuncSetAttribute(fn_dense, hipFuncAttributeMaxDynamicSharedMemorySize, (int)lds_bytes));
 		HIP_TRY(hipFuncSetAttribute(fn_wide, hipFuncAttributeMaxDynamicSharedMemorySize, (int)lds_bytes));
 		HIP_TRY(hipFuncSetAttribute(fn_compact, hipFuncAttributeMaxDynamicSharedMemorySize, (int)lds_bytes));
 		HIP_TRY(hipFuncSetAttribute((const void *)lsq_count_generic_kernel, hipFuncAttributeMaxDynamicSharedMemorySize, (int)lds_bytes));
@@ -1331,6 +1471,11 @@
 			int nb2 = 0;
 			HIP_TRY(hipOccupancyMaxActiveBlocksPerMultiprocessor(&nb, fn_wide, (int)COUNT_BLOCK, (size_t)lds_bytes));
 			HIP_TRY(hipOccupancyMaxActiveBlocksPerMultiprocessor(&nb2, fn_compact, (int)COUNT_BLOCK, (size_t)lds_bytes));
+			if (p1w == 4 && c->opt_dense_pool1 != 0) {
+				int nb3 = 0;
+				HIP_TRY(hipOccupancyMaxActiveBlocksPerMultiprocessor(&nb3, fn_dense, (int)COUNT_BLOCK, (size_t)lds_bytes));
+				nb2 = std::min(nb2, nb3);
+			}
 			c->occ_lds_bytes = lds_bytes; c->occ_p1w = p1w; c->occ_blocks = all_compact ? nb2 : std::min(nb, nb2);
 		}
 		if (c->occ_blocks >= 1) per_cu = std::min(per_cu, (unsigned)c->occ_blocks);
@@ -1397,6 +1542,8 @@
 		A.ablate = c->dev_ablate;
 		A.compact = mr.compact ? 1u : 0u;
 		A.p1 = mr.p1.p; A.p1_strand = mr.p1_strand.p; A.p1_line = mr.p1_line.p;
+		const bool dense = runs_dense(mr);
+		A.p1a = dense ? mr.p1a.p : nullptr; A.p1d = dense ? mr.p1d.p : nullptr;
 		A.p2 = mr.p2.p; A.p2_strand = mr.p2_strand.p; A.p2_line = mr.p2_line.p;
 		A.pn_blk_off = mr.pn_blk_off.p; A.pn_nblk = mr.pn_nblk.p; A.pn_se = reinterpret_cast<const int2 *>(mr.pn_se.p);
 		A.pn_strand = mr.pn_strand.p; A.pn_line = mr.pn_line.p; A.pn_bucket = mr.pn_bucket.p;
@@ -1426,7 +1573,8 @@
 			}
 #endif
 			void *kargs[] = {(void *)&A};
-			HIP_TRY(hipExtLaunchKernel(mr.compact ? fn_compact : fn_wide, fgrid, dim3(COUNT_BLOCK), kargs, lds_bytes, st, nullptr, last_streaming ? c->ev_counted2[set] : nullptr, 0));
+			if (dense) c->last_dense |= 1u << m;
+			HIP_TRY(hipExtLaunchKernel(dense ? fn_dense : (mr.compact ? fn_compact : fn_wide), fgrid, dim3(COUNT_BLOCK), kargs, lds_bytes, st, nullptr, last_streaming ? c->ev_counted2[set] : nullptr, 0));
 			if (last_streaming) counted_signalled = true;
 			if (c->time_events) HIP_TRY(hipEventRecord(c->evf1[m], st));
 			c->fast_launched |= 1 << m;
@@ -1488,6 +1636,32 @@
 	return LSQ_OK;
 } LSQ_API_CATCH
 
+int lsq_reads_dense_info(lsq_ctx *c, int method, uint64_t *groups, uint64_t *not_dense, uint64_t *mixed, int *used, uint64_t *stream_bytes) LSQ_API_TRY {
+	if (!c || method < 0 || method >= LSQ_MAX_METHODS) return fail(LSQ_E_ARG, "bad context or method");
+	const MethodReads &mr = c->reads[method];
+	if (!mr.present) return fail(LSQ_E_STATE, "no reads uploaded for method %d", method);
+	if (groups) *groups = mr.dense_groups;
+	if (not_dense) *not_dense = mr.dense_not;
+	if (mixed) *mixed = mr.dense_mixed;
+	if (stream_bytes) *stream_bytes = 24ull * mr.dense_groups;
+	if (used) *used = (c->counted && (c->last_dense >> method & 1u)) ? 1 : 0;
+	return LSQ_OK;
+} LSQ_API_CATCH
+
+int lsq_debug_dense_stream(lsq_ctx *c, int method, uint32_t *anchors, uint16_t *offsets, uint32_t *records, unsigned long long cap, unsigned long long *n) LSQ_API_TRY {
+	if (!c || !n || method < 0 || method >= LSQ_MAX_METHODS) return fail(LSQ_E_ARG, "bad argument");
+	HIP_TRY(hipSetDevice(c->device));
+	{ int rc = sync_all(c); if (rc) return rc; }
+	const MethodReads &mr = c->reads[method];
+	if (!mr.present) return fail(LSQ_E_STATE, "no reads uploaded for method %d", method);
+	const unsigned long long k = std::min<unsigned long long>(cap, mr.dense_groups);
+	if (k && anchors) HIP_TRY(hipMemcpy(anchors, mr.p1a.p, k * sizeof(uint2), hipMemcpyDeviceToHost));
+	if (k && offsets) HIP_TRY(hipMemcpy(offsets, mr.p1d.p, k * sizeof(uint4), hipMemcpyDeviceToHost));
+	if (k && records) HIP_TRY(hipMemcpy(records, mr.p1.p, 8 * k * sizeof(uint32_t), hipMemcpyDeviceToHost));
+	*n = k;
+	return LSQ_OK;
+} LSQ_API_CATCH
+
 int lsq_debug_counters(lsq_ctx *c, unsigned long long *out8) LSQ_API_TRY {
 	HIP_TRY(hipSetDevice(c->device));
 	{ int rc = sync_all(c); if (rc) return rc; }
diff --git a/lesseq_amd/csrc/lsq_device.hip b/lesseq_amd/csrc/lsq_device.hip
--- a/lesseq_amd/csrc/lsq_device.hip
+++ b/lesseq_amd/csrc/lsq_device.hip
@@ -843,6 +843,10 @@
 	} else if (n == "reads_per_look") {
 		if (!(value == 0 || value == 4 || value == 8)) return fail(LSQ_E_ARG, "reads_per_look must be 0 (automatic), 4 or 8");
 		c->opt_reads_per_look = (int)value;
+	} else if (n == "dense_pool1") {
+		if (!(value == 0 || value == 1 || value == 2)) return fail(LSQ_E_ARG, "dense_pool1 must be 0 (never), 1 (automatic) or 2 (wherever the stream exists)");
+		c->opt_dense_pool1 = (int)value;
+		c->occ_lds_bytes = 0;
 	} else if (n == "count_streams") {
 		{ int rc = sync_all(c); if (rc) return rc; }
 		c->opt_two_count_streams = value >= 2;
diff --git a/lesseq_amd/csrc/lsq_device.hpp b/lesseq_amd/csrc/lsq_device.hpp
--- a/lesseq_amd/csrc/lsq_device.hpp
+++ b/lesseq_amd/csrc/lsq_device.hpp
@@ -39,6 +39,8 @@
 constexpr unsigned COMPACT_OFF_BITS = 22, COMPACT_OFF_MASK = (1u << COMPACT_OFF_BITS) - 1u, COMPACT_MAX_LEN = 1u << 10;
 constexpr int COMPACT_BIAS = 1 << 21;
 __host__ __device__ inline bool compact_block_fits(long long off, long long len) { return off >= 0 && off <= (long long)COMPACT_OFF_MASK && len > 0 && len < (long long)COMPACT_MAX_LEN; }
+
+constexpr unsigned DENSE_PAD = 0xFFFFu, DENSE_MAX_OFF = 0xFFFEu, DENSE_MIXED = 0x8000u;
 
 struct ExcEntry {
 	unsigned long long slot;
@@ -106,6 +108,9 @@
 	uint64_t lib_report[5] = {0, 0, 0, 0, 0};
 	DevBuf<int32_t> p1, p2, pn_se;
 	bool compact = false;
+	DevBuf<uint2> p1a;
+	DevBuf<uint4> p1d;
+	uint64_t dense_groups = 0, dense_not = 0, dense_mixed = 0;
 	uint64_t n1_reads = 0, n2_reads = 0;
 	DevBuf<uint8_t> p1_strand, p2_strand, pn_strand;
 	DevBuf<uint32_t> p1_line, p2_line, pn_line, pn_blk_off, pn_nblk, pn_bucket;
@@ -154,6 +159,8 @@
 	int occ_p1w = 0;
 	int opt_reads_per_look = 0;
 	unsigned last_reads_per_look = 4, last_wg_per_cu = 0;
+	int opt_dense_pool1 = 1;
+	unsigned last_dense = 0;
 	unsigned occ_lds_bytes = 0; int occ_blocks = 0;
 	bool time_events = false;
 	bool count_timed = false, solve_timed = false;
diff --git a/lesseq_amd/csrc/lsq_ingest.hip b/lesseq_amd/csrc/lsq_ingest.hip
--- a/lesseq_amd/csrc/lsq_ingest.hip
+++ b/lesseq_amd/csrc/lsq_ingest.hip
@@ -414,6 +414,72 @@
 	}
 }
 
+__global__ void __launch_bounds__(256) lsq_ingest_dense_thresholds_kernel(const BucketDesc *buckets, const unsigned *cell_base, unsigned n_buckets, unsigned n_groups1,
+                                                                          const unsigned char *images, int2 *thr) {
+	const unsigned g = blockIdx.x * blockDim.x + threadIdx.x;
+	if (g >= n_groups1) return;
+	unsigned lo_b = 0, hi_b = n_buckets;
+	while (hi_b - lo_b > 1) { const unsigned mid = (lo_b + hi_b) >> 1; if (cell_base[mid] <= g) lo_b = mid; else hi_b = mid; }
+	const BucketDesc &d = buckets[lo_b];
+	const int base = d.lo - lsq::COMPACT_BIAS;
+	const unsigned cell = g - cell_base[lo_b];
+	int2 t = make_int2(-1, -1);
+	if (d.kind == 1u && cell < (d.iso_off & 0xFFFFu)) {
+		const lsq::Cell c = reinterpret_cast<const lsq::Cell *>(images + d.img_off + d.seg_off)[cell];
+		t = make_int2(c.e1 - base, c.e2 - base);
+	}
+	thr[g] = t;
+}
+__global__ void __launch_bounds__(256) lsq_ingest_dense_kernel(const unsigned long long *off1, unsigned n_groups1, const int2 *thr, const uint4 *p1, unsigned long long n_oct,
+                                                               uint2 *p1a, uint4 *p1d, unsigned long long *counts, const unsigned force_not) {
+	const unsigned lane = threadIdx.x & 63u;
+	const unsigned long long gsz = (unsigned long long)gridDim.x * blockDim.x;
+	for (unsigned long long o = (unsigned long long)blockIdx.x * blockDim.x + threadIdx.x; o - lane < n_oct; o += gsz) {
+		const bool on = o < n_oct;
+		bool dense = false, mixed = false;
+		if (on) {
+			unsigned lo_g = 0, hi_g = n_groups1;
+			while (hi_g - lo_g > 1) { const unsigned mid = (lo_g + hi_g) >> 1; if (off1[mid] <= o * P1_GROUP_PAD) lo_g = mid; else hi_g = mid; }
+			const int2 t = thr[lo_g];
+			const int e1 = t.x, e2 = t.y;
+			const uint4 a = p1[2 * o], b = p1[2 * o + 1];
+			const unsigned r[8] = {a.x, a.y, a.z, a.w, b.x, b.y, b.z, b.w};
+			unsigned mn = ~0u, L = ~0u, Lmax = 0u;
+#pragma unroll
+			for (int j = 0; j < 8; ++j) {
+				const unsigned len = r[j] >> lsq::COMPACT_OFF_BITS, off = r[j] & lsq::COMPACT_OFF_MASK;
+				if (!len) continue;
+				mn = min(mn, off); L = min(L, len); Lmax = max(Lmax, len);
+			}
+			unsigned h[8], top = 0u, sa = 0u, sl = 0u;
+#pragma unroll
+			for (int j = 0; j < 8; ++j) {
+				const unsigned len = r[j] >> lsq::COMPACT_OFF_BITS, off = r[j] & lsq::COMPACT_OFF_MASK;
+				h[j] = lsq::DENSE_PAD;
+				if (!len) continue;
+				h[j] = (off - mn) + (len - L);
+				top = max(top, h[j]);
+				const int e = (int)off + (int)len;
+				sa += e <= e1 ? len - L : 0u;
+				sl += e <= e2 ? len - L : 0u;
+			}
+			dense = Lmax != 0u && top <= lsq::DENSE_MAX_OFF && !(force_not && o % force_not == 0u);
+			mixed = dense && L != Lmax;
+			if (!dense) {
+#pragma unroll
+				for (int j = 0; j < 8; ++j) h[j] = lsq::DENSE_PAD;
+			}
+			p1a[o] = dense ? make_uint2(mn | (L << lsq::COMPACT_OFF_BITS), sa | (sl << 16) | (mixed ? lsq::DENSE_MIXED : 0u)) : make_uint2(r[0] & lsq::COMPACT_OFF_MASK, 0u);
+			p1d[o] = make_uint4(h[0] | (h[1] << 16), h[2] | (h[3] << 16), h[4] | (h[5] << 16), h[6] | (h[7] << 16));
+		}
+		const unsigned long long m_not = __ballot(on && !dense), m_mixed = __ballot(mixed);
+		if (lane == 0u) {
+			if (m_not) atomicAdd(&counts[0], (unsigned long long)__popcll(m_not));
+			if (m_mixed) atomicAdd(&counts[1], (unsigned long long)__popcll(m_mixed));
+		}
+	}
+}
+
 static const char *const INGEST_STAGE_NAMES[LSQ_INGEST_STAGES] = {
 	"newline_count", "route", "partition_count", "partition_scatter", "group_classify", "group_offsets", "group_place"};
 
@@ -596,6 +662,13 @@
 	mr.n1_reads = tot[4]; mr.n2_reads = tot[5];
 	if ((rc = mr.p1.alloc(mr.compact ? ((n1 + 3) & ~(size_t)3) : 2 * n1)) || (rc = mr.p1_strand.alloc(n1)) || (rc = mr.p1_line.alloc(n1))) return rc;
 	if ((rc = mr.p2.alloc(mr.compact ? 2 * ((n2 + 1) & ~(size_t)1) : 4 * n2)) || (rc = mr.p2_strand.alloc(n2)) || (rc = mr.p2_line.alloc(n2))) return rc;
+	static_assert(P1_GROUP_PAD == 8, "the dense stream holds eight 16-bit offsets per 16-byte word");
+	const size_t n_dense = mr.compact ? n1 / P1_GROUP_PAD : 0;
+	DevBuf<unsigned long long> d_dense_counts;
+	DevBuf<int2> d_dense_thr;
+	unsigned long long dense_counts[2] = {0, 0};
+	if ((rc = mr.p1a.alloc(n_dense)) || (rc = mr.p1d.alloc(n_dense)) || (rc = d_dense_counts.alloc(2)) || (rc = d_dense_thr.alloc(n_dense ? FC : 0))) return rc;
+	mr.dense_groups = 0; mr.dense_not = 0; mr.dense_mixed = 0;
 	if ((rc = mr.pn_se.alloc(2 * nnb)) || (rc = mr.pn_blk_off.alloc(nn)) || (rc = mr.pn_nblk.alloc(nn)) || (rc = mr.pn_strand.alloc(nn)) ||
 	    (rc = mr.pn_line.alloc(nn)) || (rc = mr.pn_bucket.alloc(nn))) return rc;
 	{
@@ -614,6 +687,17 @@
 			                   (const unsigned *)cnt1, (const unsigned long long *)d_off1.p, (const unsigned *)cnt2, (const unsigned long long *)d_off2.p, c->images.p,
 			                   (void *)mr.p1.p, (void *)mr.p2.p, compact, mr.p1_strand.p, mr.p1_line.p, mr.p2_strand.p, mr.p2_line.p);
 		}
+		if (n_dense) {
+			HIP_TRY(hipMemsetAsync(d_dense_counts.p, 0, 2 * sizeof(unsigned long long), st));
+			unsigned force_not = 0;
+#ifdef LSQ_DEV
+			if (const char *e = getenv("LSQ_DENSE_FORCE_NOT")) force_not = (unsigned)std::max(0l, atol(e));
+#endif
+			hipLaunchKernelGGL(lsq_ingest_dense_thresholds_kernel, dim3((unsigned)(FC / 256 + 1)), dim3(256), 0, st, c->buckets.p, c->cell_base.p, B, (unsigned)FC, c->images.p, d_dense_thr.p);
+			const unsigned dgrid = (unsigned)std::min<size_t>((n_dense + 255) / 256, (size_t)c->n_cu * 32);
+			hipLaunchKernelGGL(lsq_ingest_dense_kernel, dim3(dgrid), dim3(256), 0, st, (const unsigned long long *)d_off1.p, (unsigned)FC, (const int2 *)d_dense_thr.p,
+			                   reinterpret_cast<const uint4 *>(mr.p1.p), (unsigned long long)n_dense, mr.p1a.p, mr.p1d.p, d_dense_counts.p, force_not);
+		}
 		if (nn) {
 			NbOut N{};
 			N.ent = d_nb_ent.p; N.blk = d_nb_blk.p; N.n_ent = nb_tot[0]; N.pn_off = mr.pn_off.p; N.pnb_off = mr.pnb_off.p; N.curn = curn; N.curnb = curnb;
@@ -623,7 +707,7 @@
 			hipLaunchKernelGGL(lsq_ingest_nblock_kernel, dim3(ngrid), dim3(256), 0, st, N);
 		}
 		HIP_TRY(hipGetLastError());
-		k.end(16ull * n1p + 32ull * n2p + 4ull * (n1p + n2p) + (mr.compact ? 4ull : 8ull) * (n1 + 2 * n2) + 5ull * (n1 + n2));
+		k.end(16ull * n1p + 32ull * n2p + 4ull * (n1p + n2p) + (mr.compact ? 4ull : 8ull) * (n1 + 2 * n2) + 5ull * (n1 + n2) + 56ull * n_dense);
 	}
 	{
 		size_t want = std::max<size_t>(65536, (n1 + n2) / 4);
@@ -651,7 +735,9 @@
 		HIP_TRY(hipMemcpyAsync(f1.data(), d_off1.p, (FC + 1) * sizeof(unsigned long long), hipMemcpyDeviceToHost, st));
 		HIP_TRY(hipMemcpyAsync(f2.data(), d_off2.p, (FJ + 1) * sizeof(unsigned long long), hipMemcpyDeviceToHost, st));
 		if (FC + FJ) HIP_TRY(hipMemcpyAsync(park.data(), park1, (FC + FJ) * sizeof(unsigned), hipMemcpyDeviceToHost, st));
+		if (n_dense) HIP_TRY(hipMemcpyAsync(dense_counts, d_dense_counts.p, sizeof dense_counts, hipMemcpyDeviceToHost, st));
 		HIP_TRY(hipStreamSynchronize(st));
+		mr.dense_groups = n_dense; mr.dense_not = dense_counts[0]; mr.dense_mixed = dense_counts[1];
 		SW.mark("ingest: place + read-back");
 		stages_collect(c);
 		unsigned long long mx = 0;
@@ -818,7 +904,8 @@
 	const MethodReads &mr = c->reads[method];
 	if (!mr.present) return fail(LSQ_E_STATE, "no reads uploaded for method %d", method);
 	if (compact) *compact = mr.compact ? 1 : 0;
-	if (pool_bytes) *pool_bytes = 4ull * (mr.p1.n + mr.p2.n + mr.pn_se.n);
+	const bool dense = c->counted && (c->last_dense >> method & 1u);
+	if (pool_bytes) *pool_bytes = dense ? 24ull * mr.dense_groups + 4ull * (mr.p2.n + mr.pn_se.n) : 4ull * (mr.p1.n + mr.p2.n + mr.pn_se.n);
 	if (pool_reads) { pool_reads[0] = mr.n1_reads; pool_reads[1] = mr.n2_reads; pool_reads[2] = mr.pn_line.n; }
 	return LSQ_OK;
 } LSQ_API_CATCH
```

New measurement: 758.3 billion reads/s (median of 2 runs). About the same (+1.9%).
